# applied-ai-lab/genesis

Hardware: AMD Instinct MI355X
Metric: training images/sec (fwd+bwd+GECO step), GENESIS-V2 K=7 64x64 (higher is better)
Workload: dtype f32

## Files before the change

### genesis_amd/build.py

```python
import os
import os.path as osp
import subprocess
import sys

HERE = osp.dirname(osp.abspath(__file__))
CSRC = osp.join(HERE, 'csrc')
LIB = osp.join(HERE, 'libgenesis_hip.so')
SOURCES = ['gx_api.cpp', 'gx_comm.cpp', 'gx_conv.hip', 'gx_norm.hip', 'gx_attention.hip', 'gx_slots.hip', 'gx_optim.hip', 'gx_misc.hip', 'gx_gated.hip', 'gx_latent.hip', 'gx_dense.hip', 'gx_igemm.hip', 'gx_metrics.hip', 'gx_feed.hip', 'gx_wino.hip', 'gx_kq.hip', 'gx_bcast.hip', 'gx_sbp.hip', 'gx_wgq.hip', 'gx_wstrip.hip', 'gx_fid.hip', 'gx_tfrecord.cpp', 'gx_jpeg.cpp', 'gx_jpeg.hip', 'gx_png.cpp', 'gx_png.hip', 'gx_multid.hip']
HIPCC = os.environ.get('HIPCC', '/opt/rocm/bin/hipcc')
FLAGS = ['--offload-arch=gfx950', '-O3', '-std=c++17', '-fPIC', '-Wno-unused-value',
         '-Wno-pass-failed']


def _deps():
    d = [osp.join(CSRC, s) for s in SOURCES if osp.exists(osp.join(CSRC, s))]
    d += [osp.join(CSRC, 'gx_common.h'), osp.join(osp.dirname(HERE), 'include', 'genesis_hip.h'), osp.join(HERE, 'pk_peephole.py')]
    return d


def needs_build():
    if not osp.exists(LIB):
        return True
    t = osp.getmtime(LIB)
    return any(osp.getmtime(f) > t for f in _deps())


LLVM_BIN = os.environ.get('GENESIS_LLVM_BIN', '/opt/rocm/lib/llvm/bin')
TARGET = 'hipv4-amdgcn-amd-amdhsa--gfx950'


def _run(cmd, what):
    p = subprocess.run(cmd, stdout=subprocess.PIPE, stderr=subprocess.STDOUT)
    if p.returncode != 0:
        sys.stderr.write(' '.join(cmd) + '\n' + p.stdout.decode())
        raise RuntimeError('%s failed' % what)
    return p.stdout.decode()


def _compile_hip(src, obj):
    from genesis_amd import pk_peephole
    base = osp.splitext(obj)[0]
    asm, dev_o, hsaco, fatbin = base + '.dev.s', base + '.dev.o', base + '.hsaco', base + '.hipfb'
    _run([HIPCC] + FLAGS + ['--cuda-device-only', '-S', src, '-o', asm], 'device code generation of ' + src)
    with open(asm) as f:
        text, n = pk_peephole.rewrite(f.read())
    assert pk_peephole.count_bad(text) == 0
    with open(asm, 'w') as f:
        f.write(text)
    _run([osp.join(LLVM_BIN, 'clang'), '-x', 'assembler', '-target', 'amdgcn-amd-amdhsa', '-mcpu=gfx950', '-c', asm, '-o', dev_o],
         'assembling ' + asm)
    _run([osp.join(LLVM_BIN, 'lld'), '-flavor', 'gnu', '-m', 'elf64_amdgpu', '--no-undefined', '-shared', '-o', hsaco, dev_o],
         'linking ' + hsaco)
    _run([osp.join(LLVM_BIN, 'clang-offload-bundler'), '-type=o', '-bundle-align=4096',
          '-targets=host-x86_64-unknown-linux-gnu,' + TARGET, '-input=/dev/null', '-input=' + hsaco, '-output=' + fatbin],
         'bundling ' + fatbin)
    _run([HIPCC] + FLAGS + ['--cuda-host-only', '-Xclang', '-fcuda-include-gpubinary', '-Xclang', fatbin, '-c', src, '-o', obj],
         'host compilation of ' + src)
    for f in (asm, dev_o, hsaco, fatbin):
        os.remove(f)
    return n


def verify_objects(objs):
    from genesis_amd import pk_peephole
    import tempfile
    bad = {}
    with tempfile.TemporaryDirectory() as tmp:
        for obj in objs:
            import shutil
            shutil.copy(obj, osp.join(tmp, 'o.o'))
            subprocess.run([osp.join(LLVM_BIN, 'llvm-objdump'), '--offloading', 'o.o'], cwd=tmp, stdout=subprocess.PIPE,
                           stderr=subprocess.STDOUT)
            for f in os.listdir(tmp):
                if 'amdgcn' in f:
                    dis = subprocess.run([osp.join(LLVM_BIN, 'llvm-objdump'), '-d', osp.join(tmp, f)], stdout=subprocess.PIPE,
                                         stderr=subprocess.STDOUT)
                    n = pk_peephole.count_bad(dis.stdout.decode())
                    if n:
                        bad[osp.basename(obj)] = bad.get(osp.basename(obj), 0) + n
                os.remove(osp.join(tmp, f))
    return bad


def _jobs():
    n = os.environ.get('MAX_JOBS', '').strip()
    return max(1, int(n)) if n.isdigit() else min(16, len(SOURCES))


def build(force=False, verbose=True):
    if not force and not needs_build():
        return LIB
    from concurrent.futures import ThreadPoolExecutor
    objs, jobs = [], []
    with ThreadPoolExecutor(max_workers=_jobs()) as pool:
        for s in SOURCES:
            src = osp.join(CSRC, s)
            if not osp.exists(src):
                continue
            stem = osp.splitext(s)[0]
            obj = osp.join(CSRC, stem + ('_host.o' if s.endswith('.cpp') and stem + '.hip' in SOURCES else '.o'))
            objs.append(obj)
            if s.endswith('.hip'):
                if verbose:
                    print('%s %s -c %s -o %s   (device assembly through pk_peephole)' % (HIPCC, ' '.join(FLAGS), src, obj), flush=True)
                jobs.append((s, pool.submit(_compile_hip, src, obj)))
            else:
                cmd = [HIPCC] + FLAGS + ['-x', 'hip', '-c', src, '-o', obj]
                if verbose:
                    print(' '.join(cmd), flush=True)
                jobs.append((s, pool.submit(_run, cmd, 'hipcc on ' + s)))
        rewritten = {}
        for s, j in jobs:
            r = j.result()
            if isinstance(r, int) and r:
                rewritten[s] = r
    if verbose:
        print('pk_peephole: %d packed-fp32 instructions rewritten %s' % (sum(rewritten.values()), rewritten), flush=True)
    bad = verify_objects(objs)
    if bad:
        raise RuntimeError('affected packed-fp32 instruction forms left in the device code: %s' % bad)
    cmd = [HIPCC, '--offload-arch=gfx950', '-shared', '-fPIC', '-o', LIB] + objs + ['-ldl']
    if verbose:
        print(' '.join(cmd), flush=True)
    subprocess.check_call(cmd)
    return LIB


if __name__ == '__main__':
    print(build(force='--force' in sys.argv))
```

### genesis_amd/csrc/gx_dense.hip

```cpp
#include "gx_common.h"

namespace {

__device__ __forceinline__ float mask_factor(float m, bool elu) { return m > 0.f ? 1.f : (elu ? m + 1.f : 0.f); }

template <bool A_KC, bool B_KC, bool MASK, bool ROWSUM>
__device__ __forceinline__ void
dense_tile(float (*part)[256], float (*rpart)[16], int bx, int by, const float* __restrict__ a, int lda,
           const float* __restrict__ mask, const float* __restrict__ b, int ldb, const float* __restrict__ bias,
           int act, float* __restrict__ c, int ldc, int I, int J, int Kc, float* __restrict__ rs, int vec_a,
           int vec_b, float* __restrict__ rs2 = nullptr) {
    const int lane = threadIdx.x & 63, wave = threadIdx.x >> 6, nw = blockDim.x >> 6;
    const int idx = lane & 15, kq = lane >> 4;
    const int i0 = by * 16, j0 = bx * 16;
    const bool elu_mask = (act & 4) != 0;
    const bool acc_rs = (act & 8) != 0;
    act &= 3;
    const int ai = i0 + idx, bj = j0 + idx;
    const bool a_ok = ai < I, b_ok = bj < J;
    f32x4 acc = {0.f, 0.f, 0.f, 0.f};
    float rsum = 0.f;
#pragma unroll 2
    for (int k16 = wave * 16; k16 < Kc; k16 += nw * 16) {
        const int kb = k16 + 4 * kq;
        float av[4], bv[4];
        if (A_KC) {
            if (vec_a) {
                f32x4 t = {0.f, 0.f, 0.f, 0.f}, m = {1.f, 1.f, 1.f, 1.f};
                if (a_ok && kb < Kc) {
                    t = *reinterpret_cast<const f32x4*>(a + (size_t)ai * lda + kb);
                    if (MASK) m = *reinterpret_cast<const f32x4*>(mask + (size_t)ai * lda + kb);
                }
#pragma unroll
                for (int jj = 0; jj < 4; ++jj) av[jj] = MASK ? t[jj] * mask_factor(m[jj], elu_mask) : t[jj];
            } else {
#pragma unroll
                for (int jj = 0; jj < 4; ++jj) {
                    float t = 0.f;
                    if (a_ok && kb + jj < Kc) {
                        t = a[(size_t)ai * lda + kb + jj];
                        if (MASK) t *= mask_factor(mask[(size_t)ai * lda + kb + jj], elu_mask);
                    }
                    av[jj] = t;
                }
            }
        } else {
#pragma unroll
            for (int jj = 0; jj < 4; ++jj) {
                float t = 0.f;
                if (a_ok && kb + jj < Kc) {
                    t = a[(size_t)(kb + jj) * lda + ai];
                    if (MASK) t *= mask_factor(mask[(size_t)(kb + jj) * lda + ai], elu_mask);
                }
                av[jj] = t;
            }
        }
        if (B_KC) {
            if (vec_b) {
                f32x4 t = {0.f, 0.f, 0.f, 0.f};
                if (b_ok && kb < Kc) t = *reinterpret_cast<const f32x4*>(b + (size_t)bj * ldb + kb);
#pragma unroll
                for (int jj = 0; jj < 4; ++jj) bv[jj] = t[jj];
            } else {
#pragma unroll
                for (int jj = 0; jj < 4; ++jj)
                    bv[jj] = (b_ok && kb + jj < Kc) ? b[(size_t)bj * ldb + kb + jj] : 0.f;
            }
        } else {
#pragma unroll
            for (int jj = 0; jj < 4; ++jj)
                bv[jj] = (b_ok && kb + jj < Kc) ? b[(size_t)(kb + jj) * ldb + bj] : 0.f;
        }
#pragma unroll
        for (int jj = 0; jj < 4; ++jj) {
            acc = __builtin_amdgcn_mfma_f32_16x16x4f32(av[jj], bv[jj], acc, 0, 0, 0);
            if (ROWSUM) rsum += av[jj];
        }
    }
#pragma unroll
    for (int r = 0; r < 4; ++r) part[wave][(kq * 4 + r) * 16 + idx] = acc[r];
    if (ROWSUM) {
        rsum += __shfl_xor(rsum, 16, 64);
        rsum += __shfl_xor(rsum, 32, 64);
        if (kq == 0) rpart[wave][idx] = rsum;
    }
    __syncthreads();
    if (threadIdx.x < 256) {
        const int t = threadIdx.x;
        float s = part[0][t];
        for (int w = 1; w < nw; ++w) s += part[w][t];
        const int ci = i0 + (t >> 4), cj = j0 + (t & 15);
        if (ci < I && cj < J) {
            if (bias) s += bias[cj];
            if (act == 1) s = s > 0.f ? s : 0.f;
            if (act == 2) s += c[(size_t)ci * ldc + cj];
            if (act == 3) s = s > 0.f ? s : expm1f(s);
            c[(size_t)ci * ldc + cj] = s;
        }
    }
    if (ROWSUM && bx == 0 && threadIdx.x < 16 && i0 + (int)threadIdx.x < I) {
        float s = rpart[0][threadIdx.x];
        for (int w = 1; w < nw; ++w) s += rpart[w][threadIdx.x];
        if (acc_rs) { rs[i0 + threadIdx.x] += s; if (rs2) rs2[i0 + threadIdx.x] += s; }
        else { rs[i0 + threadIdx.x] = s; if (rs2) rs2[i0 + threadIdx.x] = s; }
    }
}

template <bool A_KC, bool B_KC, bool MASK, bool ROWSUM>
__global__ void __launch_bounds__(1024)
dense_kernel(const float* __restrict__ a, int lda, const float* __restrict__ mask, const float* __restrict__ b,
             int ldb, const float* __restrict__ bias, int act, float* __restrict__ c, int ldc, int I, int J, int Kc,
             float* __restrict__ rs, int vec_a, int vec_b, float* __restrict__ rs2) {
    __shared__ float part[16][256];
    __shared__ float rpart[16][16];
    dense_tile<A_KC, B_KC, MASK, ROWSUM>(part, rpart, blockIdx.x, blockIdx.y, a, lda, mask, b, ldb, bias, act, c, ldc,
                                         I, J, Kc, rs, vec_a, vec_b, rs2);
}

template <bool MASK, bool ROWSUM>
__global__ void __launch_bounds__(1024)
dense_bwd_pair_kernel(const float* __restrict__ g, int ldg, const float* __restrict__ y, const float* __restrict__ w,
                      const float* __restrict__ x, int ldx, float* __restrict__ dx, int lddx, int dx_act,
                      float* __restrict__ dw, float* __restrict__ db, float* __restrict__ db2, int M, int N, int K,
                      int gy_dx, int vec) {
    __shared__ float part[16][256];
    __shared__ float rpart[16][16];
    if ((int)blockIdx.y < gy_dx)
        dense_tile<true, false, MASK, false>(part, rpart, blockIdx.x, blockIdx.y, g, ldg, y, w, K, nullptr, dx_act & 7, dx,
                                             lddx, M, K, N, nullptr, vec, 0);
    else
        dense_tile<false, false, MASK, ROWSUM>(part, rpart, blockIdx.x, blockIdx.y - gy_dx, g, ldg, y, x, ldx, nullptr,
                                               (dx_act & 4) | ((dx_act & 16) ? 10 : 0), dw, K, N, K, M, db, 0, 0, db2);
}

__device__ __forceinline__ float sigmoid_f(float x) { return 1.f / (1.f + expf(-x)); }

__device__ __forceinline__ f32x4 lstm_load4(const float* p, bool coh) {
    if (!coh) return *reinterpret_cast<const f32x4*>(p);
    f32x4 v;
#pragma unroll
    for (int i = 0; i < 4; ++i) v[i] = __hip_atomic_load(p + i, __ATOMIC_RELAXED, __HIP_MEMORY_SCOPE_AGENT);
    return v;
}
__device__ __forceinline__ void lstm_store(float* p, float v, bool coh) {
    if (coh) __hip_atomic_store(p, v, __ATOMIC_RELAXED, __HIP_MEMORY_SCOPE_AGENT);
    else *p = v;
}

template <bool COH>
__device__ __forceinline__ void
lstm_fwd_body(float (&part)[4][4][256], const float* __restrict__ gx, const float* h_prev, const float* c_prev,
              const float* __restrict__ w_hh, const float* __restrict__ b_hh, int B, int H, float* act, float* c_out,
              float* h_out) {
    const int lane = threadIdx.x & 63, wave = threadIdx.x >> 6;
    const int idx = lane & 15, kq = lane >> 4;
    const int i0 = blockIdx.y * 16, j0 = blockIdx.x * 16;
    const bool a_ok = i0 + idx < B;
    f32x4 acc[4];
#pragma unroll
    for (int q = 0; q < 4; ++q) { acc[q][0] = 0.f; acc[q][1] = 0.f; acc[q][2] = 0.f; acc[q][3] = 0.f; }
    if (h_prev) {
        for (int k16 = wave * 16; k16 < H; k16 += 64) {
            const int kb = k16 + 4 * kq;
            f32x4 av = {0.f, 0.f, 0.f, 0.f};
            if (a_ok) av = lstm_load4(h_prev + (size_t)(i0 + idx) * H + kb, COH);
            f32x4 bv[4];
#pragma unroll
            for (int q = 0; q < 4; ++q)
                bv[q] = *reinterpret_cast<const f32x4*>(w_hh + (size_t)(q * H + j0 + idx) * H + kb);
#pragma unroll
            for (int jj = 0; jj < 4; ++jj)
#pragma unroll
                for (int q = 0; q < 4; ++q)
                    acc[q] = __builtin_amdgcn_mfma_f32_16x16x4f32(av[jj], bv[q][jj], acc[q], 0, 0, 0);
        }
    }
#pragma unroll
    for (int q = 0; q < 4; ++q)
#pragma unroll
        for (int r = 0; r < 4; ++r) part[wave][q][(kq * 4 + r) * 16 + idx] = acc[q][r];
    __syncthreads();
    const int t = threadIdx.x;
    const int b = i0 + (t >> 4), u = j0 + (t & 15);
    if (b < B) {
        float pre[4];
#pragma unroll
        for (int q = 0; q < 4; ++q) {
            float s = part[0][q][t];
#pragma unroll
            for (int w = 1; w < 4; ++w) s += part[w][q][t];
            pre[q] = s + gx[(size_t)b * 4 * H + q * H + u] + b_hh[q * H + u];
        }
        const float ig = sigmoid_f(pre[0]), fg = sigmoid_f(pre[1]), gg = tanhf(pre[2]), og = sigmoid_f(pre[3]);
        const float cp = c_prev ? c_prev[(size_t)b * H + u] : 0.f;
        const float cn = fg * cp + ig * gg;
        float* ar = act + (size_t)b * 4 * H + u;
        ar[0] = ig; ar[H] = fg; ar[2 * H] = gg; ar[3 * H] = og;
        c_out[(size_t)b * H + u] = cn;
        lstm_store(h_out + (size_t)b * H + u, og * tanhf(cn), COH);
    }
}

__global__ void __launch_bounds__(256)
lstm_step_fwd_kernel(const float* __restrict__ gx, const float* __restrict__ h_prev,
                     const float* __restrict__ c_prev, const float* __restrict__ w_hh,
                     const float* __restrict__ b_hh, int B, int H, float* __restrict__ act,
                     float* __restrict__ c_out, float* __restrict__ h_out) {
    __shared__ float part[4][4][256];
    lstm_fwd_body<false>(part, gx, h_prev, c_prev, w_hh, b_hh, B, H, act, c_out, h_out);
}

constexpr int kLstmSeqBar = 16;
constexpr int kLstmSeqMaxWg = 128;

__device__ __forceinline__ void lstm_grid_barrier(unsigned* bar, unsigned nwg) {
    asm volatile("s_waitcnt vmcnt(0)" ::: "memory");
    __syncthreads();
    if (threadIdx.x == 0) {
        __hip_atomic_fetch_add(bar, 1u, __ATOMIC_RELAXED, __HIP_MEMORY_SCOPE_AGENT);
        while (__hip_atomic_load(bar, __ATOMIC_RELAXED, __HIP_MEMORY_SCOPE_AGENT) < nwg) __builtin_amdgcn_s_sleep(1);
    }
    __syncthreads();
}

__device__ __forceinline__ void lstm_grid_finish(unsigned* bar, unsigned nwg) {
    if (threadIdx.x == 0) {
        const unsigned seen = __hip_atomic_fetch_add(bar + kLstmSeqBar - 1, 1u, __ATOMIC_RELAXED, __HIP_MEMORY_SCOPE_AGENT);
        if (seen == nwg - 1) {
            for (int i = 0; i < kLstmSeqBar; ++i) __hip_atomic_store(bar + i, 0u, __ATOMIC_RELAXED, __HIP_MEMORY_SCOPE_AGENT);
        }
    }
}

__global__ void __launch_bounds__(256)
lstm_seq_fwd_kernel(const float* __restrict__ gx, const float* __restrict__ w_hh, const float* __restrict__ b_hh, int T, int B,
                    int H, float* act, float* c, float* h, unsigned* bar) {
    __shared__ float part[4][4][256];
    const unsigned nwg = gridDim.x * gridDim.y;
    const size_t sh = (size_t)B * H;
    for (int t = 0; t < T; ++t) {
        if (t) lstm_grid_barrier(bar + (t - 1), nwg);
        lstm_fwd_body<true>(part, gx + (size_t)t * 4 * sh, t ? h + (size_t)(t - 1) * sh : nullptr, t ? c + (size_t)(t - 1) * sh : nullptr,
                            w_hh, b_hh, B, H, act + (size_t)t * 4 * sh, c + (size_t)t * sh, h + (size_t)t * sh);
    }
    lstm_grid_finish(bar, nwg);
}

template <bool COH>
__device__ __forceinline__ void
lstm_bwd_body(float (&part)[16][256], const float* __restrict__ g_h, const float* dgates_next, const float* __restrict__ w_hh,
              const float* __restrict__ act, const float* __restrict__ c, const float* __restrict__ c_prev, const float* dc_next,
              int B, int H, float* dgates, float* dc_prev) {
    const int lane = threadIdx.x & 63, wave = threadIdx.x >> 6, nw = blockDim.x >> 6;
    const int idx = lane & 15, kq = lane >> 4;
    const int i0 = blockIdx.y * 16, j0 = blockIdx.x * 16;
    const bool a_ok = i0 + idx < B;
    f32x4 acc = {0.f, 0.f, 0.f, 0.f};
    if (dgates_next) {
        const int Kc = 4 * H;
// ... 40 lines not shown
                     const float* __restrict__ c_prev, const float* __restrict__ dc_next, int B, int H,
                     float* __restrict__ dgates, float* __restrict__ dc_prev) {
    __shared__ float part[16][256];
    lstm_bwd_body<false>(part, g_h, dgates_next, w_hh, act, c, c_prev, dc_next, B, H, dgates, dc_prev);
}

__global__ void __launch_bounds__(1024)
lstm_seq_bwd_kernel(const float* __restrict__ g_h, const float* __restrict__ w_hh, const float* __restrict__ act,
                    const float* __restrict__ c, int T, int B, int H, float* dgates, float* dc2, unsigned* bar) {
    __shared__ float part[16][256];
    const unsigned nwg = gridDim.x * gridDim.y;
    const size_t sh = (size_t)B * H;
    for (int t = T - 1; t >= 0; --t) {
        if (t + 1 < T) lstm_grid_barrier(bar + t, nwg);
        lstm_bwd_body<true>(part, g_h + (size_t)t * sh, t + 1 < T ? dgates + (size_t)(t + 1) * 4 * sh : nullptr, w_hh,
                      act + (size_t)t * 4 * sh, c + (size_t)t * sh, t ? c + (size_t)(t - 1) * sh : nullptr,
                      t + 1 < T ? dc2 + (size_t)((t + 1) & 1) * sh : nullptr, B, H, dgates + (size_t)t * 4 * sh,
                      dc2 + (size_t)(t & 1) * sh);
    }
    lstm_grid_finish(bar, nwg);
}


constexpr int kNN_MR = 8;
__global__ void __launch_bounds__(256)
matmul_nn_fwd_kernel(const float* __restrict__ x, const float* __restrict__ w, float* __restrict__ y, int M, int N, int K) {
    const int n0 = (blockIdx.y * 256 + threadIdx.x) * 4;
    const int m0 = blockIdx.x * kNN_MR;
    if (n0 >= N) return;
    float4 acc[kNN_MR];
#pragma unroll
    for (int r = 0; r < kNN_MR; ++r) acc[r] = make_float4(0.f, 0.f, 0.f, 0.f);
    const float* xr[kNN_MR];
#pragma unroll
    for (int r = 0; r < kNN_MR; ++r) xr[r] = x + (size_t)(m0 + r < M ? m0 + r : M - 1) * K;
    for (int k = 0; k < K; ++k) {
        const float4 w4 = *reinterpret_cast<const float4*>(w + (size_t)k * N + n0);
#pragma unroll
        for (int r = 0; r < kNN_MR; ++r) {
            const float xv = xr[r][k];
            acc[r].x = fmaf(xv, w4.x, acc[r].x); acc[r].y = fmaf(xv, w4.y, acc[r].y);
            acc[r].z = fmaf(xv, w4.z, acc[r].z); acc[r].w = fmaf(xv, w4.w, acc[r].w);
        }
    }
#pragma unroll
    for (int r = 0; r < kNN_MR; ++r)
        if (m0 + r < M) *reinterpret_cast<float4*>(y + (size_t)(m0 + r) * N + n0) = acc[r];
}

constexpr int kNN_KC = 16;
__global__ void __launch_bounds__(256)
matmul_nn_dw_kernel(const float* __restrict__ x, const float* __restrict__ g, float* __restrict__ dw, int M, int N, int K) {
    __shared__ float4 red[3][kNN_KC][64];
    const int lane = threadIdx.x & 63, wave = threadIdx.x >> 6;
    const int n0 = (blockIdx.y * 64 + lane) * 4;
    const int k0 = blockIdx.x * kNN_KC;
    const bool n_ok = n0 < N;
    float4 acc[kNN_KC];
#pragma unroll
    for (int r = 0; r < kNN_KC; ++r) acc[r] = make_float4(0.f, 0.f, 0.f, 0.f);
    if (n_ok)
        for (int m = wave; m < M; m += 4) {
            const float4 g4 = *reinterpret_cast<const float4*>(g + (size_t)m * N + n0);
            const float* xm = x + (size_t)m * K;
#pragma unroll
            for (int r = 0; r < kNN_KC; ++r) {
                const float xv = xm[k0 + r < K ? k0 + r : K - 1];
                acc[r].x = fmaf(xv, g4.x, acc[r].x); acc[r].y = fmaf(xv, g4.y, acc[r].y);
                acc[r].z = fmaf(xv, g4.z, acc[r].z); acc[r].w = fmaf(xv, g4.w, acc[r].w);
            }
        }
    if (wave > 0) {
#pragma unroll
        for (int r = 0; r < kNN_KC; ++r) red[wave - 1][r][lane] = acc[r];
    }
    __syncthreads();
    if (wave == 0 && n_ok) {
#pragma unroll
        for (int r = 0; r < kNN_KC; ++r) {
            float4 v = acc[r];
#pragma unroll
            for (int w = 0; w < 3; ++w) {
                const float4 t = red[w][r][lane];
                v.x += t.x; v.y += t.y; v.z += t.z; v.w += t.w;
            }
            if (k0 + r < K) *reinterpret_cast<float4*>(dw + (size_t)(k0 + r) * N + n0) = v;
        }
    }
}

__global__ void __launch_bounds__(256)
matmul_nn_dx_kernel(const float* __restrict__ g, const float* __restrict__ w, float* __restrict__ part, int M, int N, int K,
                    int cols_per_chunk) {
    __shared__ float gs[32][68], ws[64][68];
    const int t = threadIdx.x;
    const int m0 = blockIdx.y * 32, k0 = blockIdx.z * 64;
    const int c_begin = blockIdx.x * cols_per_chunk;
    const int c_end = c_begin + cols_per_chunk < N ? c_begin + cols_per_chunk : N;
    const int mi = (t >> 4) * 2, ki = (t & 15) * 4;
    float acc[2][4] = {};
    for (int c0 = c_begin; c0 < c_end; c0 += 64) {
        for (int e = t; e < 32 * 16; e += 256) {
            const int r = e >> 4, q = (e & 15) * 4;
            float4 v = make_float4(0.f, 0.f, 0.f, 0.f);
            if (m0 + r < M && c0 + q < c_end) v = *reinterpret_cast<const float4*>(g + (size_t)(m0 + r) * N + c0 + q);
            *reinterpret_cast<float4*>(&gs[r][q]) = v;
        }
        for (int e = t; e < 64 * 16; e += 256) {
            const int r = e >> 4, q = (e & 15) * 4;
            float4 v = make_float4(0.f, 0.f, 0.f, 0.f);
            if (k0 + r < K && c0 + q < c_end) v = *reinterpret_cast<const float4*>(w + (size_t)(k0 + r) * N + c0 + q);
            *reinterpret_cast<float4*>(&ws[r][q]) = v;
        }
        __syncthreads();
#pragma unroll 4
        for (int c = 0; c < 64; c += 4) {
            float4 a[2], b[4];
#pragma unroll
            for (int i = 0; i < 2; ++i) a[i] = *reinterpret_cast<const float4*>(&gs[mi + i][c]);
#pragma unroll
            for (int j = 0; j < 4; ++j) b[j] = *reinterpret_cast<const float4*>(&ws[ki + j][c]);
#pragma unroll
            for (int i = 0; i < 2; ++i)
#pragma unroll
                for (int j = 0; j < 4; ++j)
                    acc[i][j] = fmaf(a[i].x, b[j].x, fmaf(a[i].y, b[j].y, fmaf(a[i].z, b[j].z, fmaf(a[i].w, b[j].w, acc[i][j]))));
        }
        __syncthreads();
    }
    float* o = part + (size_t)blockIdx.x * M * K;
#pragma unroll
    for (int i = 0; i < 2; ++i)
#pragma unroll
        for (int j = 0; j < 4; ++j)
            if (m0 + mi + i < M && k0 + ki + j < K) o[(size_t)(m0 + mi + i) * K + k0 + ki + j] = acc[i][j];
}

__global__ void __launch_bounds__(256)
matmul_nn_dx_reduce_kernel(const float* __restrict__ part, float* __restrict__ dx, int MK, int nchunk) {
    const int i = blockIdx.x * 256 + threadIdx.x;
    if (i >= MK) return;
    float s0 = 0.f, s1 = 0.f;
    int c = 0;
    for (; c + 1 < nchunk; c += 2) { s0 += part[(size_t)c * MK + i]; s1 += part[(size_t)(c + 1) * MK + i]; }
    if (c < nchunk) s0 += part[(size_t)c * MK + i];
    dx[i] = s0 + s1;
}

inline int matmul_nn_chunks(int N) {
    const int tiles = gx_ceil_div(N, 64);
    return tiles < 128 ? tiles : 128;
}

inline bool aligned16(const void* p) { return (reinterpret_cast<uintptr_t>(p) & 15) == 0; }
inline int dense_threads(int Kc) { return Kc >= 1024 ? 1024 : 256; }

}

extern "C" {

int gx_linear_fwd_ld(const float* x, int ldx, const float* w, const float* b, int act, float* y, int ldy, int M,
                     int N, int K, gx_stream_t stream) {
    GX_CHECK_ARG(x && w && y, "gx_linear_fwd: null pointer");
    GX_CHECK_ARG(M > 0 && N > 0 && K > 0, "gx_linear_fwd: bad M/N/K (%d,%d,%d)", M, N, K);
    GX_CHECK_ARG(ldx >= K && ldy >= N, "gx_linear_fwd: row strides (%d,%d) shorter than the rows (%d,%d)", ldx, ldy, K, N);
    GX_CHECK_ARG(act >= 0 && act <= 2, "gx_linear_fwd: act must be 0 (none), 1 (ReLU) or 2 (ELU)");
    if (act == 2) act = 3;
    hipStream_t s = (hipStream_t)stream;
    const int vec_w = (K % 4 == 0) && aligned16(w);
    const int vec_x = vec_w && (ldx % 4 == 0) && aligned16(x);
    {
        GxProf pf(KID_DENSE, s, 2.0 * M * N * K, 4.0 * ((double)M * K + (double)N * K + (double)M * N));
        hipLaunchKernelGGL((dense_kernel<true, true, false, false>), dim3(gx_ceil_div(N, 16), gx_ceil_div(M, 16)),
                           dim3(dense_threads(K)), 0, s, x, ldx, (const float*)nullptr, w, K, b, act, y, ldy, M, N, K,
                           (float*)nullptr, vec_x, vec_w, (float*)nullptr);
    }
    GX_CHECK_LAUNCH("gx_linear_fwd");
    return GX_OK;
}

int gx_linear_fwd(const float* x, const float* w, const float* b, int act, float* y, int M, int N, int K,
                  gx_stream_t stream) {
    return gx_linear_fwd_ld(x, K, w, b, act, y, N, M, N, K, stream);
}

int gx_linear_bwd_ex(const float* x, int ldx, const float* w, const float* y, const float* g, int ldg, int act,
                     float* dx, int lddx, int dx_accumulate, float* dw, float* db, float* db2, int M, int N, int K,
                     gx_stream_t stream) {
    GX_CHECK_ARG(x && w && g, "gx_linear_bwd: null pointer");
    GX_CHECK_ARG(M > 0 && N > 0 && K > 0, "gx_linear_bwd: bad M/N/K (%d,%d,%d)", M, N, K);
    GX_CHECK_ARG(ldx >= K && ldg >= N && (!dx || lddx >= K), "gx_linear_bwd: a row stride is shorter than its rows");
    GX_CHECK_ARG(act == 0 || ((act == 1 || act == 2) && y), "gx_linear_bwd: act 1 (ReLU) / 2 (ELU) needs the layer output y");
    GX_CHECK_ARG(dw || !db, "gx_linear_bwd: db is produced together with dw");
    GX_CHECK_ARG(db || !db2, "gx_linear_bwd: db2 is a second copy of db");
    hipStream_t s = (hipStream_t)stream;
    const int vec = (N % 4 == 0) && (ldg % 4 == 0) && aligned16(g) && (act == 0 || aligned16(y));
    GX_CHECK_ARG(dx_accumulate >= 0 && dx_accumulate <= 3, "gx_linear_bwd: dx_accumulate is a bit mask (1: dx, 2: dw / db)");
    const int elu = act == 2 ? 4 : 0;
    const int dwacc = (dx_accumulate & 2) ? 10 : 0;
    const int dx_act = ((dx_accumulate & 1) ? 2 : 0) | elu | ((dx_accumulate & 2) ? 16 : 0);
    if (act == 2) act = 1;
    if (dx && dw) {
        GxProf pf(KID_DENSE, s, 4.0 * M * N * K, 4.0 * (4.0 * M * N + 2.0 * N * K + 2.0 * M * K));
        const int gy_dx = gx_ceil_div(M, 16);
        const dim3 grid(gx_ceil_div(K, 16), gy_dx + gx_ceil_div(N, 16)), block(dense_threads(M > N ? M : N));
        const float* mask = act == 1 ? y : nullptr;
#define GX_PAIR(MASK, ROWSUM)                                                                                        \
        hipLaunchKernelGGL((dense_bwd_pair_kernel<MASK, ROWSUM>), grid, block, 0, s, g, ldg, mask, w, x, ldx, dx,    \
                           lddx, dx_act, dw, db, db2, M, N, K, gy_dx, vec)
        if (act == 1) { if (db) GX_PAIR(true, true); else GX_PAIR(true, false); }
        else          { if (db) GX_PAIR(false, true); else GX_PAIR(false, false); }
#undef GX_PAIR
        GX_CHECK_LAUNCH("gx_linear_bwd(dx+dw)");
        return GX_OK;
    }
    if (dx) {
        GxProf pf(KID_DENSE, s, 2.0 * M * N * K, 4.0 * (2.0 * M * N + (double)N * K + (double)M * K));
        const dim3 grid(gx_ceil_div(K, 16), gx_ceil_div(M, 16)), block(dense_threads(N));
        if (act == 1)
            hipLaunchKernelGGL((dense_kernel<true, false, true, false>), grid, block, 0, s, g, ldg, y, w, K,
                               (const float*)nullptr, dx_act & 7, dx, lddx, M, K, N, (float*)nullptr, vec, 0, (float*)nullptr);
        else
            hipLaunchKernelGGL((dense_kernel<true, false, false, false>), grid, block, 0, s, g, ldg,
                               (const float*)nullptr, w, K, (const float*)nullptr, dx_act & 7, dx, lddx, M, K, N,
                               (float*)nullptr, vec, 0, (float*)nullptr);
    }
    GX_CHECK_LAUNCH("gx_linear_bwd(dx)");
    if (dw) {
        GxProf pf(KID_DENSE, s, 2.0 * M * N * K, 4.0 * (2.0 * M * N + (double)M * K + (double)N * K));
        const dim3 grid(gx_ceil_div(K, 16), gx_ceil_div(N, 16)), block(dense_threads(M));
        if (act == 1) {
            if (db)
                hipLaunchKernelGGL((dense_kernel<false, false, true, true>), grid, block, 0, s, g, ldg, y, x, ldx,
                                   (const float*)nullptr, elu | dwacc, dw, K, N, K, M, db, 0, 0, db2);
            else
                hipLaunchKernelGGL((dense_kernel<false, false, true, false>), grid, block, 0, s, g, ldg, y, x, ldx,
                                   (const float*)nullptr, elu | dwacc, dw, K, N, K, M, (float*)nullptr, 0, 0, (float*)nullptr);
        } else {
            if (db)
                hipLaunchKernelGGL((dense_kernel<false, false, false, true>), grid, block, 0, s, g, ldg,
                                   (const float*)nullptr, x, ldx, (const float*)nullptr, dwacc, dw, K, N, K, M, db, 0, 0,
                                   db2);
            else
                hipLaunchKernelGGL((dense_kernel<false, false, false, false>), grid, block, 0, s, g, ldg,
                                   (const float*)nullptr, x, ldx, (const float*)nullptr, dwacc, dw, K, N, K, M,
                                   (float*)nullptr, 0, 0, (float*)nullptr);
        }
    }
    GX_CHECK_LAUNCH("gx_linear_bwd(dw)");
    return GX_OK;
}

int gx_linear_bwd(const float* x, const float* w, const float* y, const float* g, int act, float* dx, float* dw,
                  float* db, int M, int N, int K, gx_stream_t stream) {
    return gx_linear_bwd_ex(x, K, w, y, g, N, act, dx, K, 0, dw, db, nullptr, M, N, K, stream);
}

int gx_matmul_nn_fwd(const float* x, const float* w, float* y, int M, int N, int K, gx_stream_t stream) {
    GX_CHECK_ARG(x && w && y, "gx_matmul_nn_fwd: null pointer");
    GX_CHECK_ARG(M > 0 && N > 0 && K > 0 && (N % 4) == 0, "gx_matmul_nn_fwd: bad M/N/K (%d,%d,%d; N %% 4 == 0)", M, N, K);
    GX_CHECK_ARG(aligned16(w) && aligned16(y), "gx_matmul_nn_fwd: 16-byte alignment");
    hipStream_t s = (hipStream_t)stream;
    {
        GxProf pf(KID_DENSE, s, 2.0 * M * N * K, 4.0 * ((double)M * K + (double)N * K + (double)M * N));
        hipLaunchKernelGGL(matmul_nn_fwd_kernel, dim3(gx_ceil_div(M, kNN_MR), gx_ceil_div(N, 1024)), dim3(256), 0, s, x, w, y, M,
                           N, K);
    }
    GX_CHECK_LAUNCH("gx_matmul_nn_fwd");
    return GX_OK;
}

size_t gx_matmul_nn_bwd_ws_bytes(int M, int N, int K) {
    if (M <= 0 || N <= 0 || K <= 0) return 0;
    return (size_t)matmul_nn_chunks(N) * M * K * sizeof(float);
}

int gx_matmul_nn_bwd(const float* x, const float* w, const float* g, float* dx, float* dw, int M, int N, int K, void* ws,
                     size_t ws_bytes, gx_stream_t stream) {
    GX_CHECK_ARG(x && w && g, "gx_matmul_nn_bwd: null pointer");
    GX_CHECK_ARG(M > 0 && N > 0 && K > 0 && (N % 4) == 0, "gx_matmul_nn_bwd: bad M/N/K (%d,%d,%d; N %% 4 == 0)", M, N, K);
    GX_CHECK_ARG(aligned16(w) && aligned16(g) && (!dw || aligned16(dw)), "gx_matmul_nn_bwd: 16-byte alignment");
    hipStream_t s = (hipStream_t)stream;
    if (dw) {
        GxProf pf(KID_DENSE, s, 2.0 * M * N * K, 4.0 * ((double)M * K + (double)N * K + (double)M * N));
        hipLaunchKernelGGL(matmul_nn_dw_kernel, dim3(gx_ceil_div(K, kNN_KC), gx_ceil_div(N, 256)), dim3(256), 0, s, x, g, dw, M,
                           N, K);
        GX_CHECK_LAUNCH("gx_matmul_nn_bwd(dw)");
    }
    if (dx) {
        GX_CHECK_ARG(ws && ws_bytes >= gx_matmul_nn_bwd_ws_bytes(M, N, K), "gx_matmul_nn_bwd: workspace too small");
        const int nchunk = matmul_nn_chunks(N);
        const int cols = gx_round_up(gx_ceil_div(N, nchunk), 64);
        const int used = gx_ceil_div(N, cols);
        {
            GxProf pf(KID_DENSE, s, 2.0 * M * N * K, 4.0 * ((double)M * K + (double)N * K + (double)M * N));
            hipLaunchKernelGGL(matmul_nn_dx_kernel, dim3(used, gx_ceil_div(M, 32), gx_ceil_div(K, 64)), dim3(256), 0, s, g, w,
                               (float*)ws, M, N, K, cols);
        }
        GX_CHECK_LAUNCH("gx_matmul_nn_bwd(dx)");
        {
            GxProf pf(KID_SMALL_REDUCE, s, 0.0, 4.0 * (used + 1.0) * M * K);
            hipLaunchKernelGGL(matmul_nn_dx_reduce_kernel, dim3(gx_ceil_div(M * K, 256)), dim3(256), 0, s, (const float*)ws, dx,
                               M * K, used);
        }
        GX_CHECK_LAUNCH("gx_matmul_nn_bwd(dx reduce)");
    }
    return GX_OK;
}

// ... 76 lines not shown
```

### genesis_amd/csrc/gx_latent.hip

```cpp
#include "gx_common.h"

namespace {

constexpr float kHalfLog2Pi = 0.91893853320467274178f;

__device__ __forceinline__ float softplus_t(float x) {
    return x > 20.f ? x : log1pf(expf(x));
}
__device__ __forceinline__ float softplus_grad_t(float x) {
    if (x > 20.f) return 1.f;
    const float e = expf(x);
    return e / (e + 1.f);
}
__device__ __forceinline__ float sigmoid_t(float x) { return 1.f / (1.f + expf(-x)); }

__global__ void __launch_bounds__(256)
posterior_fwd_kernel(const float* __restrict__ zh, const float* __restrict__ eps, int B, int K, int D,
                     float* __restrict__ z, float* __restrict__ mu_o, float* __restrict__ sigma_o,
                     float* __restrict__ log_q, float* __restrict__ z2, int ldz2) {
    const int row = blockIdx.x * (blockDim.x >> 6) + (threadIdx.x >> 6);
    if (row >= K * B) return;
    const int lane = threadIdx.x & 63;
    const int k = row / B, b = row - k * B;
    const float* zr = zh + ((size_t)b * K + k) * 2 * D;
    double acc = 0.0;
    for (int d = lane; d < D; d += 64) {
        const float mu = zr[d];
        const float sg = softplus_t(zr[D + d] + 0.5f) + 1e-8f;
        const float zz = mu + sg * eps[(size_t)row * D + d];
        const float t = zz - mu;
        const float lp = -(t * t) / (2.f * (sg * sg)) - logf(sg) - kHalfLog2Pi;
        z[(size_t)row * D + d] = zz;
        if (z2) z2[(size_t)row * ldz2 + d] = zz;
        mu_o[(size_t)row * D + d] = mu;
        sigma_o[(size_t)row * D + d] = sg;
        acc += (double)lp;
    }
    acc = gx_wave_sum_d(acc);
    if (lane == 0) log_q[row] = (float)acc;
}

__global__ void __launch_bounds__(256)
posterior_bwd_kernel(const float* __restrict__ zh, const float* __restrict__ eps, const float* __restrict__ gz,
                     const float* __restrict__ gmu, const float* __restrict__ gsigma,
                     const float* __restrict__ glogq, int B, int K, int D, float* __restrict__ dzh,
                     const float* __restrict__ gz2, int ldgz2) {
    const int row = blockIdx.x * (blockDim.x >> 6) + (threadIdx.x >> 6);
    if (row >= K * B) return;
    const int lane = threadIdx.x & 63;
    const int k = row / B, b = row - k * B;
    const float* zr = zh + ((size_t)b * K + k) * 2 * D;
    float* dr = dzh + ((size_t)b * K + k) * 2 * D;
    const float gl = glogq ? glogq[row] : 0.f;
    for (int d = lane; d < D; d += 64) {
        const size_t i = (size_t)row * D + d;
        const float mu = zr[d];
        const float raw = zr[D + d] + 0.5f;
        const float sg = softplus_t(raw) + 1e-8f;
        const float e = eps[i];
        const float zz = mu + sg * e;
        const float t = zz - mu;
        const float var = sg * sg;
        const float dz = (gz ? gz[i] : 0.f) + (gz2 ? gz2[(size_t)row * ldgz2 + d] : 0.f) + gl * (-t / var);
        const float dmu = dz + gl * (t / var) + (gmu ? gmu[i] : 0.f);
        const float dsg = dz * e + gl * ((t * t) / (var * sg) - 1.f / sg) + (gsigma ? gsigma[i] : 0.f);
        dr[d] = dmu;
        dr[D + d] = dsg * softplus_grad_t(raw);
    }
}

__global__ void __launch_bounds__(256)
prior_logp_fwd_kernel(const float* __restrict__ z, const float* __restrict__ lin,
                      const float* __restrict__ log_q, int B, int K, int D, int first, float* __restrict__ log_p) {
    const int row = blockIdx.x * (blockDim.x >> 6) + (threadIdx.x >> 6);
    if (row >= K * B) return;
    const int lane = threadIdx.x & 63;
    const bool ar = lin != nullptr && row >= first;
    const float* lr = ar ? lin + (size_t)(row - first) * 2 * D : nullptr;
    double acc = 0.0;
    for (int d = lane; d < D; d += 64) {
        const float zz = z[(size_t)row * D + d];
        float lp;
        if (ar) {
            const float mu = tanhf(lr[d]);
            const float sg = sigmoid_t(lr[D + d] + 4.f) + 1e-4f;
            const float t = zz - mu;
            lp = -(t * t) / (2.f * (sg * sg)) - logf(sg) - kHalfLog2Pi;
        } else {
            lp = -(zz * zz) / 2.f - kHalfLog2Pi;
        }
        acc += (double)lp;
    }
    acc = gx_wave_sum_d(acc);
    if (lane == 0) log_p[row] = log_q ? log_q[row] - (float)acc : (float)acc;
}

__global__ void __launch_bounds__(256)
prior_sample_kernel(const float* __restrict__ lin, const float* __restrict__ eps, int B, int D, int tanh_mu,
                    float* __restrict__ z) {
    const int i = blockIdx.x * blockDim.x + threadIdx.x;
    if (i >= B * D) return;
    const int b = i / D, d = i - b * D;
    const float raw = lin[(size_t)b * 2 * D + d];
    const float mu = tanh_mu ? tanhf(raw) : raw;
    const float sg = sigmoid_t(lin[(size_t)b * 2 * D + D + d] + 4.f) + 1e-4f;
    z[i] = mu + sg * eps[i];
}

__global__ void __launch_bounds__(256)
prior_logp_bwd_kernel(const float* __restrict__ z, const float* __restrict__ lin, const float* __restrict__ glogp,
                      float sign, int B, int K, int D, int first, float* __restrict__ dz, float* __restrict__ dlin) {
    const int row = blockIdx.x * (blockDim.x >> 6) + (threadIdx.x >> 6);
    if (row >= K * B) return;
    const int lane = threadIdx.x & 63;
    const bool ar = lin != nullptr && row >= first;
    const float* lr = ar ? lin + (size_t)(row - first) * 2 * D : nullptr;
    float* dl = ar ? dlin + (size_t)(row - first) * 2 * D : nullptr;
    const float g = sign * glogp[row];
    for (int d = lane; d < D; d += 64) {
        const size_t i = (size_t)row * D + d;
        const float zz = z[i];
        if (ar) {
            const float mu = tanhf(lr[d]);
            const float s = sigmoid_t(lr[D + d] + 4.f);
            const float sg = s + 1e-4f;
            const float t = zz - mu;
            const float var = sg * sg;
            dz[i] = g * (-t / var);
            dl[d] = g * (t / var) * (1.f - mu * mu);
            dl[D + d] = g * ((t * t) / (var * sg) - 1.f / sg) * (s * (1.f - s));
        } else {
            dz[i] = g * (-zz);
        }
    }
}

__global__ void __launch_bounds__(256)
elbo_fwd_kernel(const float* __restrict__ err, const float* __restrict__ kl, const float* __restrict__ beta,
                int B, int R, float* __restrict__ out, float* __restrict__ tail, float* __restrict__ loss,
                float* __restrict__ d_err = nullptr, float* __restrict__ d_kl = nullptr) {
    __shared__ double red[2][4];
    if (d_err) {
        const float ge = 1.f / B, gk = *beta / B;
        for (int i = threadIdx.x; i < B; i += blockDim.x) d_err[i] = ge;
        if (d_kl) for (int i = threadIdx.x; i < R * B; i += blockDim.x) d_kl[i] = gk;
    }
    double se = 0.0, sk = 0.0;
    for (int i = threadIdx.x; i < B; i += blockDim.x) se += (double)err[i];
    for (int i = threadIdx.x; i < R * B; i += blockDim.x) sk += (double)kl[i];
    se = gx_wave_sum_d(se); sk = gx_wave_sum_d(sk);
    const int lane = threadIdx.x & 63, wave = threadIdx.x >> 6;
    if (lane == 0) { red[0][wave] = se; red[1][wave] = sk; }
    __syncthreads();
    if (threadIdx.x == 0) {
        const double e = ((red[0][0] + red[0][1]) + (red[0][2] + red[0][3])) / B;
        const double k = ((red[1][0] + red[1][1]) + (red[1][2] + red[1][3])) / B;
        const float ef = (float)e, kf = (float)k, bt = *beta;
        out[0] = ef + bt * kf; out[1] = ef + kf; out[2] = ef; out[3] = kf; out[4] = bt;
        if (tail) { tail[0] = ef; tail[1] = kf; }
        if (loss) loss[0] = out[0];
    }
}

__global__ void __launch_bounds__(256)
elbo_bwd_kernel(const float* __restrict__ g, const float* __restrict__ beta, int B, int R,
                float* __restrict__ d_err, float* __restrict__ d_kl) {
    const float ge = g[0] / B, gk = g[0] * (*beta) / B;
    const int i = blockIdx.x * blockDim.x + threadIdx.x;
    if (i < B) d_err[i] = ge;
    if (i < R * B) d_kl[i] = gk;
}

__global__ void __launch_bounds__(256)
pooled_head_fwd_kernel(const float* __restrict__ lin, const float* __restrict__ msum,
                       const float* __restrict__ fbias, const float* __restrict__ gamma,
                       const float* __restrict__ beta, float eps, int R, int C, float* __restrict__ y,
                       float* __restrict__ stats ) {
    const int row = blockIdx.x * (blockDim.x >> 6) + (threadIdx.x >> 6);
    if (row >= R) return;
    const int lane = threadIdx.x & 63;
    const float m = msum[row];
    const float den = m + 1e-5f;
    double s1 = 0.0, s2 = 0.0;
    for (int j = lane; j < C; j += 64) {
        const float o = (lin[(size_t)row * C + j] + m * fbias[j]) / den;
        s1 += (double)o; s2 += (double)o * o;
    }
    s1 = gx_wave_sum_d(s1); s2 = gx_wave_sum_d(s2);
    const double mean = s1 / C;
    double var = s2 / C - mean * mean;
    if (var < 0.0) var = 0.0;
    const float meanf = (float)mean, rstd = (float)(1.0 / sqrt(var + (double)eps));
    for (int j = lane; j < C; j += 64) {
        const float o = (lin[(size_t)row * C + j] + m * fbias[j]) / den;
        y[(size_t)row * C + j] = (o - meanf) * rstd * gamma[j] + beta[j];
    }
    if (lane == 0) { stats[2 * row] = meanf; stats[2 * row + 1] = rstd; }
}

__global__ void __launch_bounds__(256)
pooled_head_bwd_kernel(const float* __restrict__ lin, const float* __restrict__ msum,
                       const float* __restrict__ fbias, const float* __restrict__ gamma,
                       const float* __restrict__ stats, const float* __restrict__ g, int R, int C,
                       float* __restrict__ dlin, float* __restrict__ dmsum, float* __restrict__ cols) {
    const int row = blockIdx.x * (blockDim.x >> 6) + (threadIdx.x >> 6);
    if (row >= R) return;
    const int lane = threadIdx.x & 63;
    const float m = msum[row];
    const float den = m + 1e-5f;
    const float meanf = stats[2 * row], rstd = stats[2 * row + 1];
    double a = 0.0, b = 0.0;
    for (int j = lane; j < C; j += 64) {
        const float o = (lin[(size_t)row * C + j] + m * fbias[j]) / den;
        const float xh = (o - meanf) * rstd;
        const float dxh = g[(size_t)row * C + j] * gamma[j];
        a += (double)dxh; b += (double)dxh * xh;
    }
    a = gx_wave_sum_d(a); b = gx_wave_sum_d(b);
    const float k1 = (float)(a / C), k2 = (float)(b / C);
    double dm = 0.0;
    for (int j = lane; j < C; j += 64) {
        const float num = lin[(size_t)row * C + j] + m * fbias[j];
        const float o = num / den;
        const float xh = (o - meanf) * rstd;
        const float gv = g[(size_t)row * C + j];
        const float dobj = rstd * (gv * gamma[j] - k1 - xh * k2);
        dlin[(size_t)row * C + j] = dobj / den;
        dm += (double)dobj * ((double)fbias[j] / den - (double)num / ((double)den * den));
        float* cr = cols + (size_t)row * 3 * C;
        cr[j] = gv * xh; cr[C + j] = gv; cr[2 * C + j] = dobj * (m / den);
    }
    dm = gx_wave_sum_d(dm);
    if (lane == 0) dmsum[row] = (float)dm;
}

__global__ void __launch_bounds__(256)
pooled_head_cols_kernel(const float* __restrict__ cols, int R, int C, float* __restrict__ dgamma,
                        float* __restrict__ dbeta, float* __restrict__ dfbias) {
    __shared__ double red[8][32];
    const int cl = threadIdx.x & 31, rg = threadIdx.x >> 5;
    const int i = blockIdx.x * 32 + cl;
    double s = 0.0;
    if (i < 3 * C)
        for (int r = rg; r < R; r += 8) s += (double)cols[(size_t)r * 3 * C + i];
    red[rg][cl] = s;
    __syncthreads();
    if (rg == 0 && i < 3 * C) {
        double t = red[0][cl];
        for (int q = 1; q < 8; ++q) t += red[q][cl];
        const int which = i / C, j = i - which * C;
        (which == 0 ? dgamma : (which == 1 ? dbeta : dfbias))[j] = (float)t;
    }
}

int check_bkd(const char* name, int B, int K, int D) {
    GX_CHECK_ARG(B > 0 && K > 0 && D > 0, "%s: bad B/K/D (%d,%d,%d)", name, B, K, D);
    return GX_OK;
}

}

extern "C" {

int gx_latent_posterior_fwd(const float* zh, const float* eps, int B, int K, int D, float* z, float* mu,
                            float* sigma, float* log_q, gx_stream_t stream) {
    return gx_latent_posterior_fwd_ex(zh, eps, B, K, D, z, mu, sigma, log_q, nullptr, 0, stream);
}

int gx_latent_posterior_fwd_ex(const float* zh, const float* eps, int B, int K, int D, float* z, float* mu,
                               float* sigma, float* log_q, float* z2, int ldz2, gx_stream_t stream) {
    int rc = check_bkd("gx_latent_posterior_fwd", B, K, D);
    if (rc) return rc;
    GX_CHECK_ARG(zh && eps && z && mu && sigma && log_q, "gx_latent_posterior_fwd: null pointer");
    GX_CHECK_ARG(!z2 || ldz2 >= D, "gx_latent_posterior_fwd_ex: ldz2 (%d) < D (%d)", ldz2, D);
    hipStream_t s = (hipStream_t)stream;
    {
        GxProf pf(KID_LATENT, s, 0.0, 4.0 * (6.0 * K * B * D + K * B));
        hipLaunchKernelGGL(posterior_fwd_kernel, dim3(gx_ceil_div(K * B, 4)), dim3(256), 0, s, zh, eps, B, K, D, z,
                           mu, sigma, log_q, z2, ldz2);
    }
    GX_CHECK_LAUNCH("gx_latent_posterior_fwd");
    return GX_OK;
}

int gx_latent_posterior_bwd(const float* zh, const float* eps, const float* gz, const float* gmu,
                            const float* gsigma, const float* glogq, int B, int K, int D, float* dzh,
                            gx_stream_t stream) {
    return gx_latent_posterior_bwd_ex(zh, eps, gz, gmu, gsigma, glogq, nullptr, 0, B, K, D, dzh, stream);
}

int gx_latent_posterior_bwd_ex(const float* zh, const float* eps, const float* gz, const float* gmu,
                               const float* gsigma, const float* glogq, const float* gz2, int ldgz2, int B, int K,
                               int D, float* dzh, gx_stream_t stream) {
    int rc = check_bkd("gx_latent_posterior_bwd", B, K, D);
    if (rc) return rc;
    GX_CHECK_ARG(zh && eps && dzh, "gx_latent_posterior_bwd: null pointer");
    GX_CHECK_ARG(!gz2 || ldgz2 >= D, "gx_latent_posterior_bwd_ex: ldgz2 (%d) < D (%d)", ldgz2, D);
    hipStream_t s = (hipStream_t)stream;
    {
        GxProf pf(KID_LATENT, s, 0.0, 4.0 * (8.0 * K * B * D + K * B));
        hipLaunchKernelGGL(posterior_bwd_kernel, dim3(gx_ceil_div(K * B, 4)), dim3(256), 0, s, zh, eps, gz, gmu,
                           gsigma, glogq, B, K, D, dzh, gz2, ldgz2);
    }
    GX_CHECK_LAUNCH("gx_latent_posterior_bwd");
    return GX_OK;
}

int gx_latent_prior_logp_fwd(const float* z, const float* lin, const float* log_q, int B, int K, int D,
                             float* out, gx_stream_t stream) {
    return gx_latent_prior_logp_fwd_ex(z, lin, log_q, B, K, D, 0, out, stream);
}

int gx_latent_prior_logp_fwd_ex(const float* z, const float* lin, const float* log_q, int B, int K, int D, int all_slots,
                                float* out, gx_stream_t stream) {
    float* log_p = out;
    int rc = check_bkd("gx_latent_prior_logp_fwd", B, K, D);
    if (rc) return rc;
    GX_CHECK_ARG(z && log_p, "gx_latent_prior_logp_fwd: null pointer");
    hipStream_t s = (hipStream_t)stream;
    {
        GxProf pf(KID_LATENT, s, 0.0, 4.0 * (3.0 * K * B * D + K * B));
        hipLaunchKernelGGL(prior_logp_fwd_kernel, dim3(gx_ceil_div(K * B, 4)), dim3(256), 0, s, z, lin, log_q, B, K,
                           D, all_slots ? 0 : B, log_p);
    }
    GX_CHECK_LAUNCH("gx_latent_prior_logp_fwd");
    return GX_OK;
}

int gx_latent_prior_sample(const float* lin, const float* eps, int B, int D, float* z, gx_stream_t stream) {
    return gx_latent_prior_sample_ex(lin, eps, B, D, 1, z, stream);
}

int gx_latent_prior_sample_ex(const float* lin, const float* eps, int B, int D, int tanh_mu, float* z,
                              gx_stream_t stream) {
    GX_CHECK_ARG(lin && eps && z && B > 0 && D > 0, "gx_latent_prior_sample: bad arguments");
    hipStream_t s = (hipStream_t)stream;
    {
        GxProf pf(KID_LATENT, s, 0.0, 16.0 * B * D);
        hipLaunchKernelGGL(prior_sample_kernel, dim3(gx_ceil_div(B * D, 256)), dim3(256), 0, s, lin, eps, B, D, tanh_mu,
                           z);
    }
    GX_CHECK_LAUNCH("gx_latent_prior_sample");
    return GX_OK;
}

int gx_latent_prior_logp_bwd(const float* z, const float* lin, const float* g_out, int kl_mode, int B, int K,
                             int D, float* dz, float* dlin, gx_stream_t stream) {
    return gx_latent_prior_logp_bwd_ex(z, lin, g_out, kl_mode, B, K, D, 0, dz, dlin, stream);
}

int gx_latent_prior_logp_bwd_ex(const float* z, const float* lin, const float* g_out, int kl_mode, int B, int K,
                                int D, int all_slots, float* dz, float* dlin, gx_stream_t stream) {
    const float* glogp = g_out;
    int rc = check_bkd("gx_latent_prior_logp_bwd", B, K, D);
    if (rc) return rc;
    GX_CHECK_ARG(z && glogp && dz, "gx_latent_prior_logp_bwd: null pointer");
    GX_CHECK_ARG((lin == nullptr) == (dlin == nullptr), "gx_latent_prior_logp_bwd: lin and dlin go together");
    hipStream_t s = (hipStream_t)stream;
    {
        GxProf pf(KID_LATENT, s, 0.0, 4.0 * (6.0 * K * B * D + K * B));
        hipLaunchKernelGGL(prior_logp_bwd_kernel, dim3(gx_ceil_div(K * B, 4)), dim3(256), 0, s, z, lin, glogp,
                           kl_mode ? -1.f : 1.f, B, K, D, all_slots ? 0 : B, dz, dlin);
    }
    GX_CHECK_LAUNCH("gx_latent_prior_logp_bwd");
    return GX_OK;
}

int gx_elbo_fwd(const float* err, const float* kl, const float* beta, int B, int R, float* out, float* tail,
                float* loss, gx_stream_t stream) {
    GX_CHECK_ARG(err && beta && out, "gx_elbo_fwd: null pointer");
    GX_CHECK_ARG(B > 0 && R >= 0 && (R == 0 || kl), "gx_elbo_fwd: bad B/R (%d,%d) or missing kl", B, R);
    hipStream_t s = (hipStream_t)stream;
    {
        GxProf pf(KID_LATENT, s, 0.0, 4.0 * (B + (double)R * B));
        hipLaunchKernelGGL(elbo_fwd_kernel, dim3(1), dim3(256), 0, s, err, kl, beta, B, R, out, tail, loss);
    }
    GX_CHECK_LAUNCH("gx_elbo_fwd");
    return GX_OK;
}

int gx_elbo_fwd_grads(const float* err, const float* kl, const float* beta, int B, int R, float* out, float* tail,
                      float* loss, float* d_err, float* d_kl, gx_stream_t stream) {
    GX_CHECK_ARG(err && beta && out && d_err, "gx_elbo_fwd_grads: null pointer");
    GX_CHECK_ARG(B > 0 && R >= 0 && (R == 0 || (kl && d_kl)), "gx_elbo_fwd_grads: bad B/R (%d,%d) or missing kl / d_kl", B, R);
    hipStream_t s = (hipStream_t)stream;
    {
        GxProf pf(KID_LATENT, s, 0.0, 8.0 * (B + (double)R * B));
        hipLaunchKernelGGL(elbo_fwd_kernel, dim3(1), dim3(256), 0, s, err, kl, beta, B, R, out, tail, loss, d_err, d_kl);
    }
    GX_CHECK_LAUNCH("gx_elbo_fwd_grads");
    return GX_OK;
}

int gx_elbo_bwd(const float* g_loss, const float* beta, int B, int R, float* d_err, float* d_kl,
                gx_stream_t stream) {
    GX_CHECK_ARG(g_loss && beta && d_err, "gx_elbo_bwd: null pointer");
    GX_CHECK_ARG(B > 0 && R >= 0 && (R == 0 || d_kl), "gx_elbo_bwd: bad B/R (%d,%d) or missing d_kl", B, R);
    hipStream_t s = (hipStream_t)stream;
    const int n = R > 0 ? R * B : B;
    {
        GxProf pf(KID_LATENT, s, 0.0, 4.0 * (B + (double)R * B));
        hipLaunchKernelGGL(elbo_bwd_kernel, dim3(gx_ceil_div(n, 256)), dim3(256), 0, s, g_loss, beta, B, R, d_err,
                           d_kl);
    }
    GX_CHECK_LAUNCH("gx_elbo_bwd");
// ... 44 lines not shown
```

### genesis_amd/functions.py

```python
import os

import torch
import torch.nn.functional as F

from . import _lib
from . import autostep as _auto
from . import hip_ops as hip
from . import precision as _precision

GROUPS = 8
EPS = 1e-5

class _StepState(object):
    __slots__ = ('direct_param_grads', 'direct_written', 'async_wgrad', 'side_stream', 'keep_alive', 'early_flush')

    def __init__(self):
        self.direct_param_grads = False
        self.direct_written = set()
        self.async_wgrad = False
        self.side_stream = None
        self.keep_alive = []
        self.early_flush = None


# ... 823 lines not shown
                else:
                    dw = _wgrad_paired(h, dy, gw)
                pre = None
                if l >= 2 and hip.conv3x3_dgrad_act_supported(dy.shape[0], w.shape[1], w.shape[0], dy.shape[2], dy.shape[3]):
                    gbp = _gout(params[2 * l - 1])
                    wp = params[2 * l - 2]
                    lazy = wp.shape[0] == wp.shape[1] and _quad_ok(h.shape[0], wp.shape[1], h.shape[2], h.shape[3])
                    pre = hip.conv3x3_dgrad_act(dy, w, h, act, gbp, want_dbias=not lazy, amax_in=am, tap=True) + (gbp,)
                    am = hip.take_amax()
                else:
                    da = hip.conv3x3_dgrad(dy, w, amax_in=am)
                    am = None
            grads[2 * l], grads[2 * l + 1] = _ret(gw, dw), _ret(gb, db)
        return (dz, None, None, None) + tuple(grads)


def _quad_ok(N, C, H, W):
    return hip.conv3x3_wgrad_quad_supported(N, C, H, W)


def _wgrad_paired(h, dy, gw, gb=None):
    N, Ci, Co = h.shape[0], h.shape[1], dy.shape[1]
    if Ci == Co and hip.conv3x3_wgrad_quad_supported(N, Ci, h.shape[2], h.shape[3]):
        dw = hip.conv3x3_wgrad_quad(h, dy, out=gw, dbias_out=gb)
        return None if gw is not None else dw
    assert gb is None, 'the bias gradient rides on the four-image weight gradient only'
    if N % 2 or Ci > 32 or Co > 32 or Ci != Co or Ci % 8:
        return hip.conv3x3_wgrad(h, dy, out=gw)
    d64 = hip.conv3x3_wgrad(h.view(N // 2, 2 * Ci, *h.shape[2:]), dy.view(N // 2, 2 * Co, *dy.shape[2:]))
    dw = d64[:Co, :Ci] + d64[Co:, Ci:]
    if gw is not None:
        gw.copy_(dw)
        return None
    return dw


@ctx_bound
class MixtureWFn(torch.autograd.Function):

    @staticmethod
    def forward(ctx, x, dec, log_w, K, std1, std2, pixel_bound):
        x, dec, log_w = x.contiguous(), dec.contiguous(), log_w.contiguous()
        err, recon, x_r = hip.mixture_w_fwd(x, dec, log_w, K, std1, std2, pixel_bound)
        ctx.save_for_backward(x, dec, log_w)
        ctx.cfg = (K, std1, std2, pixel_bound)
        ctx.set_materialize_grads(False)
        return err, recon, x_r

    @staticmethod
    def backward(ctx, g_err, g_recon, g_x_r):
        x, dec, log_w = ctx.saved_tensors
        K, std1, std2, pixel_bound = ctx.cfg
        extra, extra_w = _fold_output_grads(dec, K, pixel_bound, g_recon, g_x_r, None, log_w)
        if g_err is None:
            if extra is not None:
                return None, extra, extra_w, None, None, None, None
            g_err = x.new_zeros(x.shape[0])
        ddec, dlog_w = hip.mixture_w_bwd(x, dec, log_w, g_err.contiguous(), K, std1, std2, pixel_bound)
        if extra is not None:
            ddec += extra
            if extra_w is not None:
                dlog_w += extra_w
        return None, ddec, dlog_w, None, None, None, None


def _c(t):
    return None if t is None else t.contiguous()


@ctx_bound
class PosteriorFn(torch.autograd.Function):

    @staticmethod
    def forward(ctx, zh, eps):
        zh, eps = zh.contiguous(), eps.contiguous()
        ctx.set_materialize_grads(False)
        ctx.save_for_backward(zh, eps)
        return hip.latent_posterior_fwd(zh, eps)

    @staticmethod
    def backward(ctx, gz, gmu, gsigma, glogq):
        zh, eps = ctx.saved_tensors
        return hip.latent_posterior_bwd(zh, eps, _c(gz), _c(gmu), _c(gsigma), _c(glogq)), None


@ctx_bound
class PriorLogPFn(torch.autograd.Function):

    @staticmethod
    def forward(ctx, z, lin, log_q=None, all_slots=False):
        z = z.contiguous()
        lin = None if lin is None else lin.contiguous()
        log_q = None if log_q is None else log_q.contiguous()
        ctx.save_for_backward(z, lin)
        ctx.kl_mode = log_q is not None
        ctx.all_slots = bool(all_slots)
        return hip.latent_prior_logp_fwd(z, lin, log_q, all_slots)

    @staticmethod
    def backward(ctx, g):
        z, lin = ctx.saved_tensors
        g = g.contiguous()
        dz, dlin = hip.latent_prior_logp_bwd(z, lin, g, ctx.kl_mode, ctx.all_slots)
        return dz, dlin, (g if ctx.kl_mode else None), None


@ctx_bound
class ElboFn(torch.autograd.Function):

    @staticmethod
    def forward(ctx, err, kl, beta, tail):
        err = err.contiguous()
        kl = None if kl is None else kl.contiguous()
        ctx.beta = beta
        ctx.dims = (err.numel(), 0 if kl is None else kl.numel() // err.numel())
        ctx.kl_shape = None if kl is None else kl.shape
        loss, out5 = hip.elbo_fwd(err, kl, beta, tail)
        ctx.mark_non_differentiable(out5)
        ctx.set_materialize_grads(False)
        return loss, out5

    @staticmethod
    def backward(ctx, g, _unused):
        B, R = ctx.dims
        d_err, d_kl = hip.elbo_bwd(g.contiguous(), ctx.beta, B, R)
        return d_err, (d_kl.view(ctx.kl_shape) if d_kl is not None else None), None, None


@ctx_bound
class PooledHeadFn(torch.autograd.Function):

    @staticmethod
    def forward(ctx, lin, msum, fbias, gamma, beta, eps):
        shape = lin.shape
        lin2 = lin.contiguous().view(-1, shape[-1])
        msum1 = msum.contiguous().view(-1)
        y, stats = hip.pooled_head_fwd(lin2, msum1, fbias, gamma, beta, eps)
        ctx.save_for_backward(lin2, msum1, stats)
        ctx.params = (fbias, gamma, beta)
        ctx.shapes = (shape, msum.shape)
        return y.view(shape)

    @staticmethod
    def backward(ctx, g):
        lin2, msum1, stats = ctx.saved_tensors
        fbias, gamma, beta = ctx.params
        outs = (_gout(fbias), _gout(gamma), _gout(beta))
        dlin, dmsum, dfb, dga, dbe = hip.pooled_head_bwd(lin2, msum1, fbias, gamma, stats,
                                                         g.contiguous().view(lin2.shape), out=outs)
        return (dlin.view(ctx.shapes[0]), dmsum.view(ctx.shapes[1]), _ret(outs[0], dfb), _ret(outs[1], dga),
                _ret(outs[2], dbe), None)


@ctx_bound
class SBPScanFn(torch.autograd.Function):

    @staticmethod
    def forward(ctx, logits, log_s0, last_scope):
        logits = logits.contiguous()
        log_s0 = None if log_s0 is None else log_s0.contiguous()
        ctx.save_for_backward(logits)
        ctx.last_scope = bool(last_scope)
        ctx.has_s0 = log_s0 is not None
        ctx.set_materialize_grads(False)
        return hip.sbp_scan_fwd(logits, log_s0, last_scope)

    @staticmethod
    def backward(ctx, g_m, g_s):
        logits, = ctx.saved_tensors
        want_s0 = ctx.has_s0 and ctx.needs_input_grad[1]
        g_logits, g_s0 = hip.sbp_scan_bwd(logits, _c(g_m), _c(g_s), ctx.last_scope, want_s0)
        return g_logits, g_s0, None


@ctx_bound
class CategoricalKLFn(torch.autograd.Function):

    @staticmethod
    def forward(ctx, log_m, log_m_r):
        log_m, log_m_r = log_m.contiguous(), log_m_r.contiguous()
        ctx.save_for_backward(log_m, log_m_r)
        return hip.categorical_kl_fwd(log_m, log_m_r)

    @staticmethod
    def backward(ctx, g):
        log_m, log_m_r = ctx.saved_tensors
        g_m, g_r = hip.categorical_kl_bwd(log_m, log_m_r, g.contiguous(), ctx.needs_input_grad[1])
        return g_m, g_r


@ctx_bound
class MaskReconFn(torch.autograd.Function):

    @staticmethod
    def forward(ctx, dec, log_m_r):
        ctx.save_for_backward(log_m_r)
        ctx.C = dec.shape[1]
        return log_m_r.view_as(log_m_r)

    @staticmethod
    def backward(ctx, g):
        log_m_r, = ctx.saved_tensors
        return hip.logsoftmax_k_bwd(log_m_r, g.contiguous(), ctx.C), None


@ctx_bound
class LSTMCellFn(torch.autograd.Function):

    @staticmethod
    def forward(ctx, inp, h_prev, c_prev, w_ih, w_hh, b_ih, b_hh):
        inp = inp.contiguous()
        B = inp.shape[0]
        H = w_hh.shape[1]
        gx = hip.linear_fwd(inp, w_ih, b_ih)
        act = torch.empty(B, 4 * H, device=inp.device)
        c = torch.empty(B, H, device=inp.device)
        h = torch.empty(B, H, device=inp.device)
        hp = None if h_prev is None else h_prev.contiguous()
        cp = None if c_prev is None else c_prev.contiguous()
        hip.lstm_step_fwd(gx, hp, cp, w_hh, b_hh, act, c, h)
        ctx.save_for_backward(inp, hp, cp, act, c)
        ctx.params = (w_ih, w_hh, b_ih, b_hh)
        ctx.set_materialize_grads(False)
        return h, c

    @staticmethod
    def backward(ctx, g_h, g_c):
        inp, hp, cp, act, c = ctx.saved_tensors
        w_ih, w_hh, b_ih, b_hh = ctx.params
        B, H = c.shape
        dev = inp.device
        if g_h is None:
            g_h = torch.zeros(B, H, device=dev)
        dgates = torch.empty(B, 4 * H, device=dev)
        dc_prev = torch.empty(B, H, device=dev)
        hip.lstm_step_bwd(g_h.contiguous(), None, w_hh, act, c, cp, _c(g_c), dgates, dc_prev)
        outs = [_gout_acc(p) for p in (w_ih, w_hh, b_ih, b_hh)]
        acc = outs[0][1]
        if any(o is None for o, _ in outs) or any(a != acc for _, a in outs):
            outs, acc = [(None, False)] * 4, False
        o_wih, o_whh, o_bih, o_bhh = (o for o, _ in outs)
        dinp, dw_ih, db = hip.linear_bwd(inp, w_ih, None, dgates, None, need_dx=ctx.needs_input_grad[0],
                                         out_dw=o_wih, out_db=o_bih, out_db2=o_bhh, accumulate_dw=acc)
        if hp is not None:
            dh_prev, dw_hh, _ = hip.linear_bwd(hp, w_hh, None, dgates, None, need_dx=True, need_db=False, out_dw=o_whh,
                                               accumulate_dw=acc)
        else:
            dh_prev = None
            dw_hh = torch.zeros_like(w_hh) if o_whh is None else (o_whh if acc else o_whh.zero_())
        return (dinp, dh_prev, dc_prev if cp is not None else None, _ret(o_wih, dw_ih), _ret(o_whh, dw_hh),
                _ret(o_bih, db), _ret(o_bhh, db))


@ctx_bound
class LatentSBPPosteriorFn(torch.autograd.Function):

    @staticmethod
    def forward(ctx, h, eps, w_m, b_m, w_v, b_v, w_ih, w_hh, b_ih, b_hh, w_lin, b_lin):
        h, eps = h.contiguous(), eps.contiguous()
        K, B, D = eps.shape
        F_, T, H = h.shape[1], K - 1, w_hh.shape[1]
        dev = h.device
        lin = torch.empty(K, B, 2 * D, device=dev)
        z, mu, sigma = (torch.empty(K, B, D, device=dev) for _ in range(3))
        log_q = torch.empty(K, B, device=dev)
        inp = torch.empty(max(T, 1), B, F_ + D, device=dev)
        if T:
            inp[:, :, :F_] = h
        act = torch.empty(max(T, 1), B, 4 * H, device=dev)
        c = torch.empty(max(T, 1), B, H, device=dev)
        hs = torch.empty(max(T, 1), B, H, device=dev)
        hip.linear_fwd(h, w_m, b_m, None, out=lin[0][:, :D])
        hip.linear_fwd(h, w_v, b_v, None, out=lin[0][:, D:])
        for k in range(K):
            if k:
                t = k - 1
                gx = hip.linear_fwd(inp[t], w_ih, b_ih)
                hip.lstm_step_fwd(gx, hs[t - 1] if t else None, c[t - 1] if t else None, w_hh, b_hh, act[t], c[t], hs[t])
                hip.linear_fwd(hs[t], w_lin, b_lin, None, out=lin[k])
            hip.latent_posterior_step_fwd(lin[k], eps[k], z[k], mu[k], sigma[k], log_q[k],
                                          inp[k][:, F_:] if k < T else None)
        ctx.save_for_backward(h, eps, lin, inp, act, c, hs)
        ctx.params = (w_m, b_m, w_v, b_v, w_ih, w_hh, b_ih, b_hh, w_lin, b_lin)
        ctx.set_materialize_grads(False)
        return z, mu, sigma, log_q

    @staticmethod
    def backward(ctx, gz, gmu, gsigma, glogq):
        h, eps, lin, inp, act, c, hs = ctx.saved_tensors
        w_m, b_m, w_v, b_v, w_ih, w_hh, b_ih, b_hh, w_lin, b_lin = ctx.params
        K, B, D = eps.shape
        F_, T, H = h.shape[1], K - 1, w_hh.shape[1]
        dev = h.device
        gz, gmu, gsigma, glogq = _c(gz), _c(gmu), _c(gsigma), _c(glogq)
        dlin = torch.empty(K, B, 2 * D, device=dev)
        dinp = torch.empty(max(T, 1), B, F_ + D, device=dev)
        dgates = torch.empty(max(T, 1), B, 4 * H, device=dev)
        dhs = torch.empty(B, H, device=dev)
        dc = [torch.empty(B, H, device=dev), torch.empty(B, H, device=dev)]

        def sl(g, k):
            return None if g is None else g[k]
        for k in reversed(range(K)):
            hip.latent_posterior_step_bwd(lin[k], eps[k], sl(gz, k), sl(gmu, k), sl(gsigma, k), sl(glogq, k),
                                          dinp[k][:, F_:] if k < T else None, dlin[k])
            if k:
# ... 266 lines not shown
```

### genesis_amd/genesisv2_config.py

```python
import math

import numpy as np
import torch
import torch.nn as nn
import torch.nn.functional as F
from torch.distributions.normal import Normal

from genesis_amd import autostep
from genesis_amd import compat as _compat

_compat.install()

from attrdict import AttrDict
from forge import flags

from genesis_amd import functions as fn
from genesis_amd.lazy import Lazy, LazyAttrDict, SlotList
from genesis_amd import hip_ops as hip

flags.DEFINE_integer('feat_dim', 64, 'Number of features and latents.')
flags.DEFINE_string('kernel', 'gaussian', '{laplacian, gaussian, epanechnikov')
flags.DEFINE_boolean('semiconv', True, 'Use semi-convolutional embeddings.')
flags.DEFINE_boolean('dynamic_K', False, 'Dynamic K.')
flags.DEFINE_boolean('klm_loss', False, 'KL mask regulariser.')
# ... 97 lines not shown
            sigma_init = 1.0 / (np.sqrt(K_steps) * np.log(2))
        elif kernel == 'gaussian':
            sigma_init = 1.0 / (K_steps * np.log(2))
        elif kernel == 'epanechnikov':
            sigma_init = 2.0 / K_steps
        else:
            raise ValueError('No valid kernel.')
        self.kernel = kernel
        self.colour_dim = colour_dim
        self.log_sigma = nn.Parameter(torch.tensor(sigma_init).log())
        self.semiconv = semiconv
        if semiconv:
            self.colour_head = _SemiConvParams(feat_dim, colour_dim)
        else:
            self.colour_head = nn.Conv2d(feat_dim, colour_dim, 1)


class GenesisV2(nn.Module):

    def __init__(self, cfg):
        super().__init__()
        self.K_steps = cfg.K_steps
        self.img_size = cfg.img_size
        self.pixel_bound = _cfg_get(cfg, 'pixel_bound', True)
        self.feat_dim = cfg.feat_dim
        self.klm_loss = _cfg_get(cfg, 'klm_loss', False)
        self.detach_mr_in_klm = _cfg_get(cfg, 'detach_mr_in_klm', True)
        self.dynamic_K = _cfg_get(cfg, 'dynamic_K', False)
        self.debug = _cfg_get(cfg, 'debug', False)
        self.multi_gpu = _cfg_get(cfg, 'multi_gpu', False)
        D = cfg.feat_dim
        self.encoder = _UNetParams(int(np.log2(cfg.img_size) - 1), cfg.img_size, min(D, 64), 3, D)
        self.att_process = _ICSBPParams(_cfg_get(cfg, 'kernel', 'gaussian'), self.K_steps, D,
                                        _cfg_get(cfg, 'semiconv', True))
        self.seg_head = _ConvGNReLU(D, D)
        self.feat_head = nn.Sequential(_ConvGNReLU(D, D), nn.Conv2d(D, 2 * D, 1))
        self.z_head = nn.Sequential(nn.LayerNorm(2 * D), nn.Linear(2 * D, 2 * D), nn.ReLU(inplace=True),
                                    nn.Linear(2 * D, 2 * D))
        c = D
        cm = min(c, 64)
        self.decoder_module = nn.Sequential(
            nn.Identity(),
            nn.ConvTranspose2d(D + 2, c, 5, 2, 2, 1), nn.GroupNorm(8, c), nn.ReLU(inplace=True),
            nn.ConvTranspose2d(c, c, 5, 2, 2, 1), nn.GroupNorm(8, c), nn.ReLU(inplace=True),
            nn.ConvTranspose2d(c, cm, 5, 2, 2, 1), nn.GroupNorm(8, cm), nn.ReLU(inplace=True),
            nn.ConvTranspose2d(cm, cm, 5, 2, 2, 1), nn.GroupNorm(8, cm), nn.ReLU(inplace=True),
            nn.Conv2d(cm, 4, 1))
        self.autoreg_prior = _cfg_get(cfg, 'autoreg_prior', True)
        self.prior_lstm, self.prior_linear = None, None
        if self.autoreg_prior and self.K_steps > 1:
            self.prior_lstm = nn.LSTM(D, 4 * D)
            self.prior_linear = nn.Linear(4 * D, 2 * D)
        assert _cfg_get(cfg, 'pixel_std1', 0.7) == _cfg_get(cfg, 'pixel_std2', 0.7)
        self.std = _cfg_get(cfg, 'pixel_std1', 0.7)
        self._grids = {}

    def _grid(self, device):
        key = str(device)
        if key not in self._grids:
            S, cd = self.img_size, self.att_process.colour_dim
            uv = torch.cat((torch.zeros(1, cd - 2, S, S), pixel_coords(S)), 1)[0].contiguous()
            dec_coords = pixel_coords(self.img_size // 16).contiguous()
            self._grids[key] = (uv.to(device), dec_coords.to(device))
        return self._grids[key]

    def _decoder_params(self):
        p = []
        for ci, gi in ((1, 2), (4, 5), (7, 8), (10, 11)):
            p.extend((self.decoder_module[ci].weight, self.decoder_module[ci].bias,
                      self.decoder_module[gi].weight, self.decoder_module[gi].bias))
        p.extend((self.decoder_module[13].weight, self.decoder_module[13].bias))
        return p

    def _decode(self, z_kbd, x=None, grad_through_masks=False):
        K, B, D = z_kbd.shape
        _, dec_coords = self._grid(z_kbd.device)
        dec = fn.DecoderFn.apply(z_kbd.reshape(K * B, D), dec_coords, *self._decoder_params())
        if x is None:
            x = torch.zeros(B, 3, self.img_size, self.img_size, device=z_kbd.device)
        err, recon, x_r, log_m_r = fn.MixtureFn.apply(x, dec, K, float(self.std), bool(self.pixel_bound))
        if grad_through_masks:
            log_m_r = fn.MaskReconFn.apply(dec, log_m_r)
        return err, recon, x_r, log_m_r

    def _prior_hidden(self, z_kbd):
        K, B, D = z_kbd.shape
        L = self.prior_lstm
        return fn.LSTMFn.apply(z_kbd[:-1], L.weight_ih_l0, L.weight_hh_l0, L.bias_ih_l0, L.bias_hh_l0)

    def _component_kl(self, z, log_q):
        lin = None
        if self.prior_lstm is not None:
            if z.shape[0] > 1:
                L, P = self.prior_lstm, self.prior_linear
                return fn.ARPriorKLFn.apply(z, log_q, L.weight_ih_l0, L.weight_hh_l0, L.bias_ih_l0, L.bias_hh_l0,
                                            P.weight, P.bias)
            lin = fn.linear(self._prior_hidden(z), self.prior_linear.weight, self.prior_linear.bias)
        return fn.PriorLogPFn.apply(z, lin, log_q)

    noise = None

    def forward(self, x, rand_pixel=None, eps=None, seed_idx=None):
        if x.is_cuda:
            if rand_pixel is None and eps is None and seed_idx is None:
                t = autostep.graph_forward(self, x)
                if t is not None:
                    return self._assemble(t)
            autostep.arm(self, x if (rand_pixel is None and eps is None and seed_idx is None) else None)
        return self._assemble(self._compute(x, rand_pixel, eps, seed_idx))

    def _compute(self, x, rand_pixel=None, eps=None, seed_idx=None):
        B, _, H, W = x.shape
        K, D = self.K_steps, self.feat_dim
        dev = x.device
        uv, _ = self._grid(dev)
        enc_feat = fn.UNetEncoderFn.apply(x, self.encoder.num_blocks, 8, *self.encoder.flat_params())
        if rand_pixel is None and eps is None and getattr(self, 'noise', None) is not None:
            rand_pixel, eps = self.noise((B, 1, H, W), (K, B, D), dev)
        if rand_pixel is None:
            rand_pixel = torch.rand(B, 1, H, W, device=dev)
        ap = self.att_process
        if ap.semiconv:
            cw, cb, gate, addend = ap.colour_head.conv.weight, ap.colour_head.conv.bias, ap.colour_head.gate.gate, uv
        else:
            cw, cb, gate, addend = ap.colour_head.weight, ap.colour_head.bias, None, None
        seg_params = self.seg_head.params()
        min_mass = 20.0 if self.dynamic_K else 0.0
        f = None
        if fn.heads_pairable(enc_feat, seg_params[0], cw, self.feat_head[0].params()[0]):
            res = fn.SegFeatHeadsFn.apply(enc_feat, *seg_params, cw, cb, gate, addend, ap.log_sigma, rand_pixel, K,
                                          ap.kernel, seed_idx, min_mass, *self.feat_head[0].params())
            res, f = res[:-1], res[-1]
        elif fn.seg_head_fusable(enc_feat, seg_params[0], cw):
            res = fn.SegICSBPFn.apply(enc_feat, *seg_params, cw, cb, gate, addend, ap.log_sigma, rand_pixel, K, ap.kernel,
                                      seed_idx, min_mass)
        else:
            seg = fn.ConvGNReLUFn.apply(enc_feat, *seg_params)
            res = fn.ICSBPFn.apply(seg, cw, cb, gate, addend, ap.log_sigma, rand_pixel, K, ap.kernel, seed_idx, min_mass)
        log_m, log_s, colour, seeds, idx = res[:5]
        dyn_batched = False
        if self.dynamic_K:
            if B == 1:
                n = int(res[5][0])
                K = n + 1
                log_m, log_s = log_m[:K], log_s[:K]
                seeds, idx = seeds[:min(n + 1, self.K_steps - 1)], idx[:min(n + 1, self.K_steps - 1)]
                if eps is not None:
                    eps = eps[:K]
            else:
                dyn_batched = True
        if f is None:
            f = fn.ConvGNReLUFn.apply(enc_feat, *self.feat_head[0].params())
        S, msum = fn.MaskPoolFn.apply(f, log_m)
        ln = self.z_head[0]
        zh = fn.PooledHeadFn.apply(fn.linear(S, self.feat_head[1].weight), msum, self.feat_head[1].bias,
                                   ln.weight, ln.bias, ln.eps)
        if eps is None:
            eps = torch.randn(K, B, D, device=dev)
        zh = fn.linear(zh, self.z_head[1].weight, self.z_head[1].bias, 'relu')
        zh = fn.linear(zh, self.z_head[3].weight, self.z_head[3].bias)
        z, mu, sigma, log_q = fn.PosteriorFn.apply(zh, eps)
        err, recon, x_r, log_m_r = self._decode(z, x, self.klm_loss and not self.detach_mr_in_klm)
        kl = self._component_kl(z, log_q)
        t = dict(err=err, kl=kl, recon=recon, log_m=log_m, log_s=log_s, x_r=x_r, log_m_r=log_m_r, colour=colour, seeds=seeds,
                 idx=idx, mu=mu, sigma=sigma, z=z)
        if self.klm_loss:
            t['kl_m'] = fn.CategoricalKLFn.apply(log_m, log_m_r.detach() if self.detach_mr_in_klm else log_m_r)
        t['dyn_batched'] = dyn_batched
        return t

    def _assemble(self, t):
        err, kl, recon, log_m, log_s, x_r, log_m_r = t['err'], t['kl'], t['recon'], t['log_m'], t['log_s'], t['x_r'], t['log_m_r']
        colour, seeds, idx, mu, sigma, z, dyn_batched = t['colour'], t['seeds'], t['idx'], t['mu'], t['sigma'], t['z'], t['dyn_batched']
        ap = self.att_process
        uv, _ = self._grid(recon.device)
        losses = AttrDict()
        losses['err'] = err
        log_m_k = list(log_m.unbind(0))
        log_s_k = None if dyn_batched else list(log_s.unbind(0))
        x_r_k = list(x_r.unbind(0))
        log_m_r_k = list(log_m_r.unbind(0))
        if 'kl_m' in t:
            losses['kl_m'] = t['kl_m']
        losses['kl_l_k'] = SlotList(kl.unbind(0), stacked=kl)

        stats = LazyAttrDict(
            recon=recon, log_m_k=log_m_k, log_s_k=log_s_k, x_r_k=x_r_k, log_m_r_k=log_m_r_k,
            mx_r_k=Lazy(lambda: list((x_r * log_m_r.exp()).unbind(0))),
            instance_seg=Lazy(lambda: torch.argmax(log_m.squeeze(2), dim=0)),
            instance_seg_r=Lazy(lambda: torch.argmax(log_m_r.squeeze(2), dim=0)))
        att_stats = LazyAttrDict()
        att_stats.update({'colour': colour,
                          'delta': Lazy(lambda: colour[:, -2:] - uv[-2:]) if ap.semiconv else None,
                          'seeds': list(seeds.unbind(0)), 'seed_idx': list(idx.unbind(0))})
        comp_stats = AttrDict(mu_k=list(mu.unbind(0)), sigma_k=list(sigma.unbind(0)), z_k=list(z.unbind(0)),
                              kl_l_k=[], q_z_k=[Normal(m, s, validate_args=False)
                                                for m, s in zip(mu.unbind(0), sigma.unbind(0))])
        if self.multi_gpu:
            del comp_stats['q_z_k']
        if dyn_batched:
            att_stats = None
        return recon, losses, stats, att_stats, comp_stats

    def decode_latents(self, z_k):
        _, recon, x_r, log_m_r = self._decode(torch.stack(list(z_k), 0))
        return recon, list(x_r.unbind(0)), list(log_m_r.unbind(0))

    @torch.no_grad()
    def sample(self, batch_size, K_steps=None, eps=None):
        K_steps = self.K_steps if K_steps is None else K_steps
        dev = self.decoder_module[13].weight.device
        D = self.feat_dim
        if eps is None:
            eps = torch.randn(K_steps, batch_size, D, device=dev)
        eps = eps.to(dev).contiguous()
        assert eps.shape == (K_steps, batch_size, D)
        if self.autoreg_prior and self.prior_lstm is not None:
            z_k = [eps[0]]
            w_ih, w_hh = self.prior_lstm.weight_ih_l0, self.prior_lstm.weight_hh_l0
            b_ih, b_hh = self.prior_lstm.bias_ih_l0, self.prior_lstm.bias_hh_l0
            H = w_hh.shape[1]
            h_prev = c_prev = None
            for k in range(1, K_steps):
                gx = hip.linear_fwd(z_k[-1].contiguous(), w_ih, b_ih)
                act = torch.empty(batch_size, 4 * H, device=dev)
                c = torch.empty(batch_size, H, device=dev)
                h = torch.empty(batch_size, H, device=dev)
                hip.lstm_step_fwd(gx, h_prev, c_prev, w_hh, b_hh, act, c, h)
                lin = hip.linear_fwd(h, self.prior_linear.weight, self.prior_linear.bias)
                z_k.append(hip.latent_prior_sample(lin, eps[k]))
                h_prev, c_prev = h, c
        else:
            z_k = list(eps.unbind(0))
        recon, x_r_k, log_m_r_k = self.decode_latents(z_k)
        stats = AttrDict(x_k=x_r_k, log_m_k=log_m_r_k, mx_k=[x * m.exp() for x, m in zip(x_r_k, log_m_r_k)],
                         z_k=z_k)
        return recon, stats

    def get_features(self, image_batch):
        with torch.no_grad():
            _, _, _, _, comp_stats = self.forward(image_batch)
            return torch.cat(comp_stats.z_k, dim=1)
```

### genesis_amd/hip_ops.py

```python
import ctypes
import os

import torch

from . import _lib
from ._lib import GenesisHipError

F32 = torch.float32
KERNELS = {'gaussian': 0, 'laplacian': 1, 'epanechnikov': 2}


def _chk(t, name, dtype=F32):
    if t is None:
        return
    if not t.is_cuda:
        raise GenesisHipError('%s: the HIP hot path needs device tensors (got %s); there is no CPU fallback'
                              % (name, t.device))
    if t.dtype != dtype:
        raise GenesisHipError('%s: expected %s, got %s' % (name, dtype, t.dtype))
    if not t.is_contiguous():
        raise GenesisHipError('%s: tensor must be contiguous' % name)


def _p(t):
# ... 1072 lines not shown
    _chk(z, 'prior.z'); _chk(lin, 'prior.lin'); _chk(log_q, 'prior.log_q')
    K, B, D = z.shape
    if lin is not None and tuple(lin.shape) != (K if all_slots else K - 1, B, 2 * D):
        raise GenesisHipError('latent_prior_logp_fwd: lin must be [%s,B,2D]' % ('K' if all_slots else 'K-1'))
    out = torch.empty(K, B, dtype=F32, device=z.device)
    _lib.call('gx_latent_prior_logp_fwd_ex', _p(z), _p(lin), _p(log_q), B, K, D, int(bool(all_slots)), _p(out), _stream())
    return out


def latent_prior_sample(lin, eps, tanh_mu=True):
    _chk(lin, 'prior_sample.lin'); _chk(eps, 'prior_sample.eps')
    B, D = eps.shape
    assert lin.shape == (B, 2 * D)
    z = torch.empty(B, D, dtype=F32, device=eps.device)
    _lib.call('gx_latent_prior_sample_ex', _p(lin), _p(eps), B, D, int(bool(tanh_mu)), _p(z), _stream())
    return z


def latent_prior_logp_bwd(z, lin, g_out, kl_mode=False, all_slots=False):
    _chk(g_out, 'prior_bwd.g_out')
    K, B, D = z.shape
    dz = torch.empty_like(z)
    dlin = torch.empty_like(lin) if lin is not None else None
    _lib.call('gx_latent_prior_logp_bwd_ex', _p(z), _p(lin), _p(g_out), int(kl_mode), B, K, D, int(bool(all_slots)), _p(dz),
              _p(dlin), _stream())
    return dz, dlin


def elbo_fwd(err, kl, beta, tail=None):
    _chk(err, 'elbo.err'); _chk(kl, 'elbo.kl'); _chk(beta, 'elbo.beta'); _chk(tail, 'elbo.tail')
    B = err.numel()
    R = 0 if kl is None else kl.numel() // B
    out = torch.empty(5, dtype=F32, device=err.device)
    loss = torch.empty(1, dtype=F32, device=err.device)
    _lib.call('gx_elbo_fwd', _p(err), _p(kl), _p(beta), B, R, _p(out), _p(tail), _p(loss), _stream())
    return loss, out


def elbo_fwd_grads(err, kl, beta, tail=None):
    _chk(err, 'elbo.err'); _chk(kl, 'elbo.kl'); _chk(beta, 'elbo.beta'); _chk(tail, 'elbo.tail')
    B = err.numel()
    R = 0 if kl is None else kl.numel() // B
    out = torch.empty(5, dtype=F32, device=err.device)
    d_err = torch.empty_like(err)
    d_kl = torch.empty_like(kl) if kl is not None else None
    _lib.call('gx_elbo_fwd_grads', _p(err), _p(kl), _p(beta), B, R, _p(out), _p(tail), None, _p(d_err), _p(d_kl), _stream())
    return out, d_err, d_kl


def elbo_bwd(g_loss, beta, B, R):
    _chk(g_loss, 'elbo_bwd.g')
    d_err = torch.empty(B, dtype=F32, device=g_loss.device)
    d_kl = torch.empty(R, B, dtype=F32, device=g_loss.device) if R else None
    _lib.call('gx_elbo_bwd', _p(g_loss), _p(beta), B, R, _p(d_err), _p(d_kl), _stream())
    return d_err, d_kl


def pooled_head_fwd(lin, msum, fbias, gamma, beta, eps):
    for t, n in ((lin, 'lin'), (msum, 'msum'), (fbias, 'fbias'), (gamma, 'gamma'), (beta, 'beta')):
        _chk(t, 'pooled_head.' + n)
    R, C = lin.shape
    y = torch.empty_like(lin)
    stats = torch.empty(R, 2, dtype=F32, device=lin.device)
    _lib.call('gx_pooled_head_fwd', _p(lin), _p(msum), _p(fbias), _p(gamma), _p(beta), float(eps), R, C, _p(y),
              _p(stats), _stream())
    return y, stats


def pooled_head_bwd(lin, msum, fbias, gamma, stats, g, out=(None, None, None)):
    _chk(g, 'pooled_head_bwd.g')
    R, C = lin.shape
    dev = lin.device
    dlin = torch.empty_like(lin)
    dmsum = torch.empty(R, dtype=F32, device=dev)
    dfb, dga, dbe = [o if o is not None else torch.empty(C, dtype=F32, device=dev) for o in out]
    nb = _lib.query('gx_pooled_head_bwd_ws_bytes', R, C)
    ws = _ws(nb, dev)
    _lib.call('gx_pooled_head_bwd', _p(lin), _p(msum), _p(fbias), _p(gamma), _p(stats), _p(g), R, C, _p(dlin),
              _p(dmsum), _p(dfb), _p(dga), _p(dbe), _p(ws), ws.numel(), _stream())
    return dlin, dmsum, dfb, dga, dbe


def _rows(t, name):
    if t.dim() != 2 or t.stride(1) != 1 or t.stride(0) < t.shape[1] or t.dtype != F32 or not t.is_cuda:
        raise GenesisHipError('%s: needs a float32 device matrix with contiguous rows, got %s strides %s'
                              % (name, tuple(t.shape), tuple(t.stride())))
    return t.stride(0)


def bcast_deconv_pack(w, b, coords):
    _chk(w, 'bcast_deconv.w'); _chk(b, 'bcast_deconv.b'); _chk(coords, 'bcast_deconv.coords')
    D, Cout, d = w.shape[0] - 2, w.shape[1], coords.shape[-1]
    if tuple(w.shape[2:]) != (5, 5) or coords.numel() != 2 * d * d or D <= 0:
        raise GenesisHipError('bcast_deconv_pack: w %s / coords %s' % (tuple(w.shape), tuple(coords.shape)))
    rows = Cout * 4 * d * d
    wz = torch.empty(rows, D, dtype=F32, device=w.device)
    bias = torch.empty(rows, dtype=F32, device=w.device)
    _lib.call('gx_bcast_deconv5x5s2_pack', _p(w), _p(b), _p(coords), D, Cout, d, _p(wz), _p(bias), _stream())
    return wz, bias


def bcast_deconv_unpack(dwz, dbias, coords, Cout, out_dw=None, out_db=None, want_db=False):
    _chk(dwz, 'bcast_deconv.dwz'); _chk(dbias, 'bcast_deconv.dbias'); _chk(coords, 'bcast_deconv.coords')
    _chk(out_dw, 'bcast_deconv.out_dw'); _chk(out_db, 'bcast_deconv.out_db')
    D, d = dwz.shape[1], coords.shape[-1]
    dw = out_dw if out_dw is not None else torch.empty(D + 2, Cout, 5, 5, dtype=F32, device=dwz.device)
    db = out_db if out_db is not None else (torch.empty(Cout, dtype=F32, device=dwz.device) if want_db else None)
    _lib.call('gx_bcast_deconv5x5s2_unpack', _p(dwz), _p(dbias), _p(coords), D, Cout, d, _p(dw), _p(db), _stream())
    return dw, db


def linear_fwd(x, w, b=None, act=None, out=None):
    _chk(w, 'linear.w'); _chk(b, 'linear.b')
    ldx = _rows(x, 'linear.x')
    M, K = x.shape
    N = w.shape[0]
    if w.shape[1] != K:
        raise GenesisHipError('linear_fwd: x is [%d,%d] but w is %s' % (M, K, tuple(w.shape)))
    y = torch.empty(M, N, dtype=F32, device=x.device) if out is None else out
    ldy = _rows(y, 'linear.out')
    if tuple(y.shape) != (M, N):
        raise GenesisHipError('linear_fwd: out is %s, expected (%d, %d)' % (tuple(y.shape), M, N))
    _lib.call('gx_linear_fwd_ld', _p(x), ldx, _p(w), _p(b), ACTS[act], _p(y), ldy, M, N, K, _stream())
    _probe_act(y, b, act)
    return y


def linear_bwd(x, w, y, g, act=None, need_dx=True, need_dw=True, need_db=True, out_dw=None, out_db=None,
               out_db2=None, accumulate_dx=None, accumulate_dw=False, out_dx=None):
    assert not accumulate_dw or out_dw is not None
    M, K = x.shape
    N = w.shape[0]
    dev = x.device
    ldx, ldg = _rows(x, 'linear_bwd.x'), _rows(g, 'linear_bwd.g')
    if y is not None and _rows(y, 'linear_bwd.y') != ldg:
        raise GenesisHipError('linear_bwd: y and g must share a row stride')
    if accumulate_dx is not None:
        dx = accumulate_dx
    elif out_dx is not None:
        dx = out_dx
    else:
        dx = torch.empty(M, K, dtype=F32, device=dev) if need_dx else None
    if dx is not None and tuple(dx.shape) != (M, K):
        raise GenesisHipError('linear_bwd: dx is %s, expected (%d, %d)' % (tuple(dx.shape), M, K))
    lddx = _rows(dx, 'linear_bwd.dx') if dx is not None else K
    dw = (out_dw if out_dw is not None else torch.empty(N, K, dtype=F32, device=dev)) if need_dw else None
    db = (out_db if out_db is not None else torch.empty(N, dtype=F32, device=dev)) if (need_db and need_dw) else None
    _lib.call('gx_linear_bwd_ex', _p(x), ldx, _p(w), _p(y), _p(g), ldg, ACTS[act], _p(dx), lddx,
              int(accumulate_dx is not None) | (2 if accumulate_dw else 0), _p(dw), _p(db),
              _p(out_db2 if db is not None else None), M, N, K, _stream())
    return dx, dw, db


def matmul_nn_fwd(x, w):
    _chk(x, 'matmul_nn.x'); _chk(w, 'matmul_nn.w')
    M, K = x.shape
    if w.shape[0] != K:
        raise GenesisHipError('matmul_nn_fwd: x is [%d,%d] but w is %s' % (M, K, tuple(w.shape)))
    y = torch.empty(M, w.shape[1], dtype=F32, device=x.device)
    _lib.call('gx_matmul_nn_fwd', _p(x), _p(w), _p(y), M, w.shape[1], K, _stream())
    return y


def matmul_nn_bwd(x, w, g, need_dx=True, out_dw=None, need_dw=True):
    _chk(x, 'matmul_nn_bwd.x'); _chk(w, 'matmul_nn_bwd.w'); _chk(g, 'matmul_nn_bwd.g')
    M, K = x.shape
    N = w.shape[1]
    dx = torch.empty(M, K, dtype=F32, device=x.device) if need_dx else None
    dw = (out_dw if out_dw is not None else torch.empty(K, N, dtype=F32, device=x.device)) if need_dw else None
    nb = _lib.query('gx_matmul_nn_bwd_ws_bytes', M, N, K) if need_dx else 0
    ws = _ws(nb, x.device) if need_dx else None
    _lib.call('gx_matmul_nn_bwd', _p(x), _p(w), _p(g), _p(dx), _p(dw), M, N, K, _p(ws), nb, _stream())
    return dx, dw


def logsoftmax_k_fwd(dec, K):
    _chk(dec, 'logsoftmax_k_fwd.dec')
    KB, C, H, W = dec.shape
    B = KB // K
    out = torch.empty(K, B, 1, H, W, dtype=F32, device=dec.device)
    _lib.call('gx_logsoftmax_k_fwd', _p(dec), K, B, H * W, C, _p(out), _stream())
    return out


def lstm_step_fwd(gx, h_prev, c_prev, w_hh, b_hh, act, c, h):
    B, H4 = gx.shape
    for t, n in ((gx, 'gx'), (h_prev, 'h_prev'), (c_prev, 'c_prev'), (w_hh, 'w_hh'), (b_hh, 'b_hh'), (act, 'act'),
                 (c, 'c'), (h, 'h')):
        _chk(t, 'lstm_step_fwd.' + n)
    _lib.call('gx_lstm_step_fwd', _p(gx), _p(h_prev), _p(c_prev), _p(w_hh), _p(b_hh), B, H4 // 4, _p(act), _p(c),
              _p(h), _stream())


def lstm_step_bwd(g_h, dgates_next, w_hh, act, c, c_prev, dc_next, dgates, dc_prev):
    B, H4 = act.shape
    for t, n in ((g_h, 'g_h'), (dgates_next, 'dgates_next'), (act, 'act'), (c, 'c'), (c_prev, 'c_prev'),
                 (dc_next, 'dc_next'), (dgates, 'dgates'), (dc_prev, 'dc_prev')):
        _chk(t, 'lstm_step_bwd.' + n)
    _lib.call('gx_lstm_step_bwd', _p(g_h), _p(dgates_next), _p(w_hh), _p(act), _p(c), _p(c_prev), _p(dc_next), B,
              H4 // 4, _p(dgates), _p(dc_prev), _stream())


LSTM_SEQ = os.environ.get('GENESIS_LSTM_SEQ', '0') == '1'
_LSTM_BAR = {}


def _lstm_bar(device, which):
    key = (device.index, torch.cuda.current_stream(device).cuda_stream, which)
    t = _LSTM_BAR.get(key)
    if t is None:
        t = _LSTM_BAR[key] = torch.zeros(_lib.query('gx_lstm_seq_ws_bytes') // 4, dtype=torch.int32, device=device)
    return t


def lstm_seq_steps(B, H):
    return lstm_seq_capacity(B, H) if LSTM_SEQ else 0


def lstm_seq_capacity(B, H):
    return _lib.query('gx_lstm_seq_max_steps', B, H)


def lstm_seq_fwd(gx3, w_hh, b_hh, act, c, h):
    T, B, H4 = gx3.shape
    for t, n in ((gx3, 'gx'), (w_hh, 'w_hh'), (b_hh, 'b_hh'), (act, 'act'), (c, 'c'), (h, 'h')):
        _chk(t, 'lstm_seq_fwd.' + n)
    _lib.call('gx_lstm_seq_fwd', _p(gx3), _p(w_hh), _p(b_hh), T, B, H4 // 4, _p(act), _p(c), _p(h),
              _p(_lstm_bar(gx3.device, 0)), _stream())


def lstm_seq_bwd(g_h, w_hh, act, c, dgates, dc2):
    T, B, H4 = act.shape
    for t, n in ((g_h, 'g_h'), (w_hh, 'w_hh'), (act, 'act'), (c, 'c'), (dgates, 'dgates'), (dc2, 'dc2')):
        _chk(t, 'lstm_seq_bwd.' + n)
    _lib.call('gx_lstm_seq_bwd', _p(g_h), _p(w_hh), _p(act), _p(c), T, B, H4 // 4, _p(dgates), _p(dc2),
              _p(_lstm_bar(act.device, 1)), _stream())


def conv1x1_gn_fwd(y_pre, mean, rstd, gamma, beta, groups, w, bias, gate=None, addend=None):
    _chk(y_pre, 'conv1x1_gn.y'); _chk(mean, 'conv1x1_gn.mean'); _chk(rstd, 'conv1x1_gn.rstd')
    _chk(gamma, 'conv1x1_gn.gamma'); _chk(beta, 'conv1x1_gn.beta'); _chk(w, 'conv1x1_gn.w'); _chk(bias, 'conv1x1_gn.bias')
    _chk(gate, 'conv1x1_gn.gate'); _chk(addend, 'conv1x1_gn.addend')
    N, Cin, H, W = y_pre.shape
    Cout = w.shape[0]
    out = torch.empty(N, Cout, H, W, dtype=F32, device=y_pre.device)
    _lib.call('gx_conv1x1_gn_fwd', _p(y_pre), _p(mean), _p(rstd), _p(gamma), _p(beta), groups, _p(w), _p(bias),
              _p(gate), _p(addend), N, Cin, Cout, H, W, _p(out), _stream())
    return out


def conv1x1_gn_wgrad(y_pre, mean, rstd, gamma, beta, groups, g_out, w=None, bias=None, gate=None, out=None):
    _chk(y_pre, 'conv1x1_gn_wgrad.y'); _chk(g_out, 'conv1x1_gn_wgrad.g')
    N, Cin, H, W = y_pre.shape
    Cout = g_out.shape[1]
    o = out or (None, None, None)
    dw = o[0] if o[0] is not None else torch.empty(Cout, Cin, dtype=F32, device=y_pre.device)
    db = o[1] if o[1] is not None else torch.empty(Cout, dtype=F32, device=y_pre.device)
    dgate = (o[2] if o[2] is not None else torch.empty((), dtype=F32, device=y_pre.device)) if gate is not None else None
    _chk(dw, 'conv1x1_gn_wgrad.dw'); _chk(db, 'conv1x1_gn_wgrad.db'); _chk(dgate, 'conv1x1_gn_wgrad.dgate')
    assert dw.numel() == Cout * Cin and db.numel() == Cout
    nb = _lib.query('gx_conv1x1_gn_wgrad_ws_bytes', N, Cin, Cout, H, W)
    ws = _ws(nb, y_pre.device)
    _lib.call('gx_conv1x1_gn_wgrad', _p(y_pre), _p(mean), _p(rstd), _p(gamma), _p(beta), groups, _p(g_out), _p(w),
              _p(bias), _p(gate), N, Cin, Cout, H, W, _p(dw), _p(db), _p(dgate), _p(ws), nb, _stream())
    return dw, db, dgate


def conv1x1_gn_bwd_fused(y, gamma, beta, mean, rstd, groups, g_out, w, bias, gate=None, want_dbias=False,
                         out_gn=None, out_conv=None):
    N, C, H, W = y.shape
    Cout = int(g_out.shape[1])
    if not _lib.query('gx_gn_relu_bwd_proj_fuses_wgrad', C, H, W, groups, Cout):
        return None
    wpart = torch.empty(N, Cout, C, dtype=F32, device=y.device)
    bpart = torch.empty(N, Cout, dtype=F32, device=y.device)
    dy, dgamma, dbeta, dbias = gn_relu_bwd_proj(y, gamma, beta, mean, rstd, groups, g_out, w, want_dbias, out_gn, gate,
                                                parts=(wpart, bpart))
    o = out_conv or (None, None, None)
    dw = o[0] if o[0] is not None else torch.empty(Cout, C, dtype=F32, device=y.device)
    db = o[1] if o[1] is not None else torch.empty(Cout, dtype=F32, device=y.device)
    dgate = (o[2] if o[2] is not None else torch.empty((), dtype=F32, device=y.device)) if gate is not None else None
    _chk(dw, 'conv1x1_gn_bwd.dw'); _chk(db, 'conv1x1_gn_bwd.db'); _chk(dgate, 'conv1x1_gn_bwd.dgate')
    assert dw.numel() == Cout * C and db.numel() == Cout
    nb = _lib.query('gx_conv1x1_gn_wgrad_finish_ws_bytes', C, Cout)
    ws = _ws(nb, y.device)
    _lib.call('gx_conv1x1_gn_wgrad_finish', _p(wpart), _p(bpart), N, C, Cout, _p(w), _p(bias), _p(gate), _p(dw), _p(db),
              _p(dgate), _p(ws), nb, _stream())
    return dy, (dgamma, dbeta, dbias), (dw, db, dgate)


def gn_relu_bwd_proj(y, gamma, beta, mean, rstd, groups, g_out, w, want_dbias=False, out=None, gate=None,
                     parts=(None, None)):
    _chk(y, 'gn_bwd_proj.y'); _chk(g_out, 'gn_bwd_proj.g'); _chk(w, 'gn_bwd_proj.w')
    N, C, H, W = y.shape
    dy = torch.empty_like(y)
    o = out or (None, None, None)
    dgamma = o[0] if o[0] is not None else torch.empty(C, dtype=F32, device=y.device)
    dbeta = o[1] if o[1] is not None else torch.empty(C, dtype=F32, device=y.device)
    dbias = (o[2] if o[2] is not None else torch.empty(C, dtype=F32, device=y.device)) if want_dbias else None
    nb = _lib.query('gx_gn_relu_bwd_proj_ws_bytes', N, C, H, W, groups, int(g_out.shape[1]))
    ws = _ws(nb, y.device)
    direct = o[0] is not None and o[1] is not None and (not want_dbias or o[2] is not None)
    tap = _tap_begin(y.device, H * W, y.numel())
    with _deferring(direct, ws):
        _lib.call('gx_gn_relu_bwd_proj', _p(y), _p(gamma), _p(beta), _p(mean), _p(rstd), N, C, H, W, groups,
                  _p(g_out), int(g_out.shape[1]), _p(w), _p(gate), _p(dy), _p(dgamma), _p(dbeta), _p(dbias),
# ... 61 lines not shown
```

### include/genesis_hip.h

```cpp
#ifndef GENESIS_HIP_H
#define GENESIS_HIP_H
#include <stddef.h>
#include <stdint.h>

#ifdef __cplusplus
extern "C" {
#endif

typedef void* gx_stream_t;

#define GX_OK 0
#define GX_EINVAL (-1)
#define GX_ELAUNCH (-2)
#define GX_EDATA (-3)

const char* gx_last_error(void);
int gx_version(void);

size_t gx_conv3x3_ws_bytes(int N, int Cin, int Cout, int H, int W);
int gx_conv3x3_fwd(const float* x, const float* w, float* y, int N, int Cin, int Cout, int H, int W,
                   void* ws, size_t ws_bytes, gx_stream_t stream);
int gx_conv3x3_dgrad(const float* dy, const float* w, float* dx, int N, int Cin, int Cout, int H, int W,
                     void* ws, size_t ws_bytes, gx_stream_t stream);
int gx_conv3x3_dgrad_parts(const float* dy, const float* w, float* dx, int N, int Cin, int Cout, int H, int W, void* ws,
// ... 146 lines not shown
int gx_profile_enable(int on);
int gx_profile_num_kernels(void);
const char* gx_profile_kernel_name(int kid);
int gx_profile_collect(double* total_ms, double* launches, double* flops, double* bytes);

int gx_conv3x3_bias_act_fwd(const float* x, const float* w, const float* bias, int act, float* y, int N, int Cin,
                            int Cout, int H, int W, void* ws, size_t ws_bytes, gx_stream_t stream);
size_t gx_bias_act_bwd_ws_bytes(int N, int C);
int gx_bias_act_bwd(const float* out, const float* g, int N, int C, int H, int W, int act, float* dy, float* dbias,
                    void* ws, size_t ws_bytes, gx_stream_t stream);
int gx_conv3x3_dgrad_act_supported(int N, int Cin, int Cout, int H, int W);
size_t gx_conv3x3_dgrad_act_ws_bytes(int N, int Cin, int Cout, int H, int W);
int gx_conv3x3_dgrad_act(const float* dy, const float* w, const float* xout, int act, float* dxa, float* dbias, int N,
                         int Cin, int Cout, int H, int W, void* ws, size_t ws_bytes, gx_stream_t stream);
int gx_conv3x3_wgrad_quad_supported(int N, int C, int H, int W);
size_t gx_conv3x3_wgrad_quad_ws_bytes(int N, int C, int H, int W);
int gx_conv3x3_wgrad_quad(const float* x, const float* dy, float* dw, int N, int C, int H, int W, void* ws, size_t ws_bytes,
                          gx_stream_t stream);
size_t gx_conv3x3_wgrad_quad_bias_ws_bytes(int N, int C, int H, int W);
int gx_conv3x3_wgrad_quad_bias(const float* x, const float* dy, float* dw, float* dbias, int N, int C, int H, int W, void* ws,
                               size_t ws_bytes, gx_stream_t stream);
int gx_conv5x5s1_supported(int N, int K, int M, int H, int W);
size_t gx_conv5x5s1_ws_bytes(int N, int K, int M, int H, int W);
int gx_conv5x5s1(const float* in, const float* w, float* out, int N, int K, int M, int H, int W, int flip, void* ws,
                 size_t ws_bytes, gx_stream_t stream);
int gx_conv5x5_wgrad_supported(int N, int CA, int CB, int H, int W);
size_t gx_conv5x5_wgrad_ws_bytes(int N, int CA, int CB, int H, int W);
int gx_conv5x5_wgrad(const float* a, const float* b, float* dw, int N, int CA, int CB, int H, int W, void* ws,
                     size_t ws_bytes, gx_stream_t stream);

int gx_conv3x3s2_dgrad_small(const float* dy, const float* w, float* dx, int N, int Cin, int Cout, int H, int W, int cin_n,
                             gx_stream_t stream);
int gx_conv3x3s2_dgrad_small_ex(const float* dy, const float* w, float* dx, int N, int Cin, int Cout, int H, int W, int cin_n,
                                int dx_channels, gx_stream_t stream);
int gx_mask_image_stack(const float* mask, const float* x, float* out, int K, int B, int C, int H, int W, gx_stream_t stream);
size_t gx_conv3x3s2_wgrad_small_ws_bytes(int N, int Cin, int Cout, int H, int W);
int gx_conv3x3s2_wgrad_small(const float* x, const float* dy, float* dw, int N, int Cin, int Cout, int H, int W, void* ws,
                             size_t ws_bytes, gx_stream_t stream);
int gx_conv2d_direct_fwd(const float* x, const float* w, const float* bias, int act, float* y, int N, int Cin,
                         int Cout, int H, int W, int k, int stride, int pad, gx_stream_t stream);
size_t gx_conv2d_direct_fwd_ws_bytes(int N, int Cin, int Cout, int H, int W, int k, int stride, int pad);
int gx_conv2d_direct_fwd_ws(const float* x, const float* w, const float* bias, int act, float* y, int N, int Cin,
                            int Cout, int H, int W, int k, int stride, int pad, void* ws, size_t ws_bytes,
                            gx_stream_t stream);
int gx_conv2d_direct_dgrad(const float* dy, const float* w, float* dx, int N, int Cin, int Cout, int H, int W, int k,
                           int stride, int pad, gx_stream_t stream);
size_t gx_conv2d_direct_wgrad_ws_bytes(int N, int Cin, int Cout, int H, int W, int k, int stride, int pad);
int gx_conv2d_direct_wgrad(const float* x, const float* dy, float* dw, int N, int Cin, int Cout, int H, int W, int k,
                           int stride, int pad, void* ws, size_t ws_bytes, gx_stream_t stream);
int gx_mixture_w_fwd(const float* x, const float* dec, const float* log_w, int dec_ch, int B, int H, int W, int K,
                     float pixel_std1, float pixel_std2, int pixel_bound, float* recon, float* x_r, float* err,
                     void* ws, size_t ws_bytes, gx_stream_t stream);
int gx_mixture_w_bwd(const float* x, const float* dec, const float* log_w, const float* g_err, int dec_ch, int B,
                     int H, int W, int K, float pixel_std1, float pixel_std2, int pixel_bound, float* ddec,
                     float* dlog_w, gx_stream_t stream);

size_t gx_gated_stats_floats(int norm, int N, int C);
int gx_gated_norm_fwd(const float* y, const float* bias, int norm, const float* gamma_h, const float* beta_h,
                      const float* gamma_g, const float* beta_g, int N, int C, int H, int W, float eps, float* out,
                      float* stats, gx_stream_t stream);
int gx_bn_running_update(const float* stats, int C, double m, float eps, float momentum, float* rm_h, float* rv_h, float* rm_g,
                         float* rv_g, long long* nbt_h, long long* nbt_g, gx_stream_t stream);
int gx_gated_bn_running(float* rm_h, float* rv_h, float* rm_g, float* rv_g, long long* nbt_h, long long* nbt_g, float momentum);
size_t gx_gated_norm_bwd_ws_bytes(int norm, int N, int C);
int gx_gated_norm_bwd(const float* y, const float* bias, int norm, const float* gamma_h, const float* beta_h,
                      const float* gamma_g, const float* beta_g, const float* stats, const float* dout, int N, int C,
                      int H, int W, float* dy, float* dgamma_h, float* dbeta_h, float* dgamma_g, float* dbeta_g,
                      float* dbias, void* ws, size_t ws_bytes, gx_stream_t stream);

size_t gx_gated_bn_sums_ws_bytes(int N, int C);
int gx_gated_bn_local_sums(const float* y, const float* bias, int N, int C, int H, int W, double* sums, void* ws,
                           size_t ws_bytes, gx_stream_t stream);
int gx_gated_bn_apply(const float* y, const float* bias, const double* sums, double m, const float* gamma_h,
                      const float* beta_h, const float* gamma_g, const float* beta_g, int N, int C, int H, int W, float eps,
                      float* out, float* stats, gx_stream_t stream);
int gx_gated_bn_bwd_local_sums(const float* y, const float* bias, const float* gamma_h, const float* beta_h,
                               const float* gamma_g, const float* beta_g, const float* stats, const float* dout, int N, int C,
                               int H, int W, float* sums, float* dgamma_h, float* dbeta_h, float* dgamma_g, float* dbeta_g,
                               float* dbias, void* ws, size_t ws_bytes, gx_stream_t stream);
int gx_gated_bn_bwd_apply(const float* y, const float* bias, const float* gamma_h, const float* beta_h, const float* gamma_g,
                          const float* beta_g, const float* stats, const float* dout, const float* sums, double m, int N, int C,
                          int H, int W, float* dy, gx_stream_t stream);

int gx_sbp_scan_fwd(const float* logits, const float* log_s0, int T, size_t P, int last_scope, float* log_m,
                    float* log_s, gx_stream_t stream);
int gx_sbp_scan_bwd(const float* logits, const float* g_log_m, const float* g_log_s, int T, size_t P, int last_scope,
                    float* g_logits, float* g_log_s0, gx_stream_t stream);
int gx_categorical_kl_fwd(const float* log_m, const float* log_m_r, int K, int B, int HW, float* kl,
                          gx_stream_t stream);
int gx_categorical_kl_bwd(const float* log_m, const float* log_m_r, const float* g_kl, int K, int B, int HW,
                          float* g_log_m, float* g_log_m_r, gx_stream_t stream);
int gx_logsoftmax_k_fwd(const float* dec, int K, int B, int HW, int C, float* log_m_r, gx_stream_t stream);
int gx_logsoftmax_k_bwd(const float* log_m_r, const float* g, int K, int B, int HW, int C, float* g_dec,
                        gx_stream_t stream);

int gx_broadcast_concat(const float* z, const float* coords, float* out, int N, int D, int d, gx_stream_t stream);
int gx_bcast_deconv5x5s2_pack(const float* w, const float* b, const float* coords, int D, int Cout, int d, float* wz,
                              float* bias, gx_stream_t stream);
int gx_bcast_deconv5x5s2_unpack(const float* dwz, const float* dbias, const float* coords, int D, int Cout, int d,
                                float* dw, float* db, gx_stream_t stream);
int gx_bcast_conv3x3_fwd(const float* z, const float* w, const float* bias, const float* rowc, const float* colc,
                         int act, float* out, int N, int L, int Co, int d, gx_stream_t stream);
size_t gx_bcast_conv3x3_bwd_ws_bytes(int N, int Co);
int gx_bcast_conv3x3_bwd(const float* y, const float* g, const float* z, const float* w, const float* rowc,
                         const float* colc, int act, int N, int L, int Co, int d, float* dz, float* dw, float* db,
                         void* ws, size_t ws_bytes, gx_stream_t stream);

int gx_latent_posterior_fwd(const float* zh, const float* eps, int B, int K, int D, float* z, float* mu,
                            float* sigma, float* log_q, gx_stream_t stream);
int gx_latent_posterior_bwd(const float* zh, const float* eps, const float* gz, const float* gmu,
                            const float* gsigma, const float* glogq, int B, int K, int D, float* dzh,
                            gx_stream_t stream);
int gx_latent_posterior_fwd_ex(const float* zh, const float* eps, int B, int K, int D, float* z, float* mu,
                               float* sigma, float* log_q, float* z2, int ldz2, gx_stream_t stream);
int gx_latent_posterior_bwd_ex(const float* zh, const float* eps, const float* gz, const float* gmu,
                               const float* gsigma, const float* glogq, const float* gz2, int ldgz2, int B, int K,
                               int D, float* dzh, gx_stream_t stream);
int gx_latent_prior_logp_fwd(const float* z, const float* lin, const float* log_q, int B, int K, int D,
                             float* out, gx_stream_t stream);
int gx_latent_prior_logp_bwd(const float* z, const float* lin, const float* g_out, int kl_mode, int B, int K,
                             int D, float* dz, float* dlin, gx_stream_t stream);
int gx_latent_prior_logp_fwd_ex(const float* z, const float* lin, const float* log_q, int B, int K, int D, int all_slots,
                                float* out, gx_stream_t stream);
int gx_latent_prior_logp_bwd_ex(const float* z, const float* lin, const float* g_out, int kl_mode, int B, int K,
                                int D, int all_slots, float* dz, float* dlin, gx_stream_t stream);
int gx_latent_prior_sample(const float* lin, const float* eps, int B, int D, float* z, gx_stream_t stream);
int gx_latent_prior_sample_ex(const float* lin, const float* eps, int B, int D, int tanh_mu, float* z,
                              gx_stream_t stream);

int gx_elbo_fwd(const float* err, const float* kl, const float* beta, int B, int R, float* out, float* tail,
                float* loss, gx_stream_t stream);
int gx_elbo_fwd_grads(const float* err, const float* kl, const float* beta, int B, int R, float* out, float* tail,
                      float* loss, float* d_err, float* d_kl, gx_stream_t stream);
int gx_elbo_bwd(const float* g_loss, const float* beta, int B, int R, float* d_err, float* d_kl,
                gx_stream_t stream);

int gx_pooled_head_fwd(const float* lin, const float* msum, const float* fbias, const float* gamma,
                       const float* beta, float eps, int R, int C, float* y, float* stats, gx_stream_t stream);
size_t gx_pooled_head_bwd_ws_bytes(int R, int C);
int gx_pooled_head_bwd(const float* lin, const float* msum, const float* fbias, const float* gamma,
                       const float* stats, const float* g, int R, int C, float* dlin, float* dmsum, float* dfbias,
                       float* dgamma, float* dbeta, void* ws, size_t ws_bytes, gx_stream_t stream);

int gx_linear_fwd(const float* x, const float* w, const float* b, int act, float* y, int M, int N, int K,
                  gx_stream_t stream);
int gx_linear_bwd(const float* x, const float* w, const float* y, const float* g, int act, float* dx, float* dw,
                  float* db, int M, int N, int K, gx_stream_t stream);
int gx_linear_fwd_ld(const float* x, int ldx, const float* w, const float* b, int act, float* y, int ldy, int M,
                     int N, int K, gx_stream_t stream);
int gx_linear_bwd_ex(const float* x, int ldx, const float* w, const float* y, const float* g, int ldg, int act,
                     float* dx, int lddx, int dx_accumulate, float* dw, float* db, float* db2, int M, int N, int K,
                     gx_stream_t stream);

int gx_matmul_nn_fwd(const float* x, const float* w, float* y, int M, int N, int K, gx_stream_t stream);
size_t gx_matmul_nn_bwd_ws_bytes(int M, int N, int K);
int gx_matmul_nn_bwd(const float* x, const float* w, const float* g, float* dx, float* dw, int M, int N, int K,
                     void* ws, size_t ws_bytes, gx_stream_t stream);

int gx_lstm_step_fwd(const float* gx, const float* h_prev, const float* c_prev, const float* w_hh,
                     const float* b_hh, int B, int H, float* act, float* c, float* h, gx_stream_t stream);
int gx_lstm_step_bwd(const float* g_h, const float* dgates_next, const float* w_hh, const float* act,
                     const float* c, const float* c_prev, const float* dc_next, int B, int H, float* dgates,
                     float* dc_prev, gx_stream_t stream);
int gx_lstm_seq_max_steps(int B, int H);
size_t gx_lstm_seq_ws_bytes(void);
int gx_lstm_seq_fwd(const float* gx, const float* w_hh, const float* b_hh, int T, int B, int H, float* act, float* c,
                    float* h, void* bar, gx_stream_t stream);
int gx_lstm_seq_bwd(const float* g_h, const float* w_hh, const float* act, const float* c, int T, int B, int H,
                    float* dgates, float* dc2, void* bar, gx_stream_t stream);

int gx_weight_cache_create(void);
int gx_weight_cache_record(int id, int on);
int gx_weight_cache_size(int id);
int gx_weight_cache_refresh(int id, gx_stream_t stream);
int gx_weight_cache_release(void);
int gx_weight_cache_activate(int id);
int gx_weight_cache_destroy(int id);

int gx_ctx_create(void);
int gx_ctx_make_current(int id);
int gx_ctx_current(void);
int gx_ctx_destroy(int id);

int gx_defer_enable(int on);
int gx_defer_pending(void);
int gx_defer_flush(gx_stream_t stream);

int gx_conv3x3_fwd_parts(const float* x, const float* w, float* y, int N, int Cin, int Cout, int H, int W, void* ws,
                         size_t ws_bytes, const float** parts, int* nsplit, size_t* split_stride, gx_stream_t stream);
int gx_deconv5x5s2_fwd_parts(const float* x, const float* w, float* y, int N, int Cin, int Cout, int Hin, int Win,
                             void* ws, size_t ws_bytes, const float** parts, int* nsplit, size_t* split_stride,
                             gx_stream_t stream);
int gx_gn_relu_fwd_parts(const float* parts, int nsplit, size_t split_stride, const float* conv_bias, float* y_sum,
                         const float* gamma, const float* beta, int N, int C, int H, int W, int groups, float eps,
                         float* dst0, int dst0_ctot, int dst0_c0, int dst0_mode, float* dst1, int dst1_ctot,
                         int dst1_c0, int dst1_mode, float* mean, float* rstd, gx_stream_t stream);

int gx_label_contingency(const long long* segA, const long long* segB, int B, int HW, int KA, int KB, int* counts,
                         gx_stream_t stream);

#define GX_FID_MAXPOOL_S2 0
#define GX_FID_MAXPOOL_S1P1 1
#define GX_FID_AVGPOOL_S1P1 2
#define GX_FID_GLOBAL_AVGPOOL 3
int gx_fid_preprocess(const float* x, float* y, int B, int H, int W, int quantise, gx_stream_t stream);
int gx_fid_conv_bias_relu(const float* x, int B, int H, int W, int Cin, const float* w, const float* bias, int kh, int kw,
                          int stride, int ph, int pw, float* d0, int d0_ctot, int d0_c0, int n0, float* d1, int d1_ctot,
                          int d1_c0, int n1, float* d2, int d2_ctot, int d2_c0, int n2, gx_stream_t stream);
int gx_fid_pool(const float* x, int B, int H, int W, int C, int mode, float* y, int y_ctot, int y_c0, gx_stream_t stream);
int gx_fid_moments(const float* feats, int B, int D, double* sum, double* sumsq, gx_stream_t stream);

int gx_u8hwc_to_f32chw(const unsigned char* src, float* dst, int B, int Hs, int Ws, int C, int H, int W,
                       gx_stream_t stream);

#define GX_RESAMPLE_NEAREST 0
#define GX_RESAMPLE_PIL_BILINEAR 1
#define GX_LABEL_U8 0
#define GX_LABEL_I32 1
#define GX_LABEL_I64 2
int gx_pil_bilinear_ksize(int in, int out);
int gx_pil_bilinear_coeffs(int in, int out, int ksize, int* bounds, int* weights);
int gx_u8hwc_resample_f32chw(const unsigned char* src, float* dst, int B, int Hs, int Ws, int C, int top, int left, int Hc,
                             int Wc, int H, int W, int mode, const int* hbounds, const int* hweights, int hksize,
                             const int* vbounds, const int* vweights, int vksize, gx_stream_t stream);
int gx_labels_crop_nearest(const void* src, int dtype, long long* dst, int B, int Hs, int Ws, int top, int left, int Hc, int Wc,
                           int H, int W, gx_stream_t stream);

#define GX_ROWS_U8 0
#define GX_ROWS_F32 1
#define GX_LABEL_F32 3
#define GX_LABEL_F64 4
int gx_rows_gather_f32chw(const void* src, int dtype, long long N, const long long* idx, long long idx_len, long long first,
                          float* dst, int B, int Hs, int Ws, int C, int H, int W, gx_stream_t stream);
int gx_rows_gather_labels(const void* src, int dtype, long long N, const long long* idx, long long idx_len, long long first,
                          long long* dst, int B, int Hs, int Ws, int H, int W, gx_stream_t stream);
int gx_sprites_compose(const unsigned char* sprites, int S, const int* first, const int* count, const unsigned char* colours,
                       float* img, unsigned char* mask, int n, gx_stream_t stream);

unsigned int gx_crc32c(const void* data, size_t n);
unsigned int gx_crc32c_masked(const void* data, size_t n);
int gx_tfrecord_scan(const unsigned char* buf, size_t n, int verify_crc, long long first_index, int max_records,
                     long long* offsets, long long* lengths, int* num_records, size_t* consumed);
int gx_tfexample_find_bytes_list(const unsigned char* rec, size_t n, const char* name, long long* offset, long long* length);
int gx_bytes_list_unpack(const unsigned char* payload, size_t n, unsigned char* dst, size_t expected);
int gx_entity_masks_to_labels(const unsigned char* masks, long long* dst, int B, int E, int Hs, int Ws, long long entity_stride,
                              long long pixel_stride, int background_entities, int top, int left, int Hc, int Wc, int H, int W,
                              gx_stream_t stream);

int gx_bytes_list_index(const unsigned char* payload, size_t n, int max_values, long long* offsets, long long* lengths, int* count);
int gx_jpeg_info(const unsigned char* data, size_t len, int* info);
int gx_jpeg_entropy_decode(const unsigned char* data, size_t len, short* coef, size_t coef_capacity, unsigned short* qtab,
                           int* info);
int gx_jpeg_decode_f32chw(const short* coef, const unsigned short* qtab, float* dst_f32, unsigned char* dst_u8, int B, int H, int W,
                          int sampling, int S_h, int S_w, gx_stream_t stream);

#define GX_PNG_PLANE_BYTE 0
#define GX_PNG_PLANE_SHAPESTACKS_REF 1
#define GX_PNG_PLANE_INDEX 2
int gx_png_info(const unsigned char* data, size_t len, int* info);
int gx_png_inflate(const unsigned char* data, size_t len, unsigned char* dst, size_t dst_capacity, int* info);
int gx_png_unfilter(const unsigned char* filtered, unsigned char* dst_u8, unsigned char* dst_plane0, int plane_rule, int B, int H,
                    int W, int C, gx_stream_t stream);

size_t gx_allreduce_unique_id_bytes(void);
int gx_allreduce_unique_id(void* id, size_t id_bytes);
int gx_allreduce_init(const void* id, size_t id_bytes, int rank, int world, void** comm);
int gx_allreduce_run(void* comm, float* buf, size_t count, gx_stream_t stream);
int gx_allreduce_destroy(void* comm);

int gx_mfma_fp32_probe(int wgs, int iters, int mode, float* scratch, double* flops, gx_stream_t stream);

#ifdef __cplusplus
}
#endif
#endif
```

Before: 12290.

## Fuse slot posterior head into single forward and batched backward kernels

Adds a fused slot-head path that runs the pooled feature linear, layer norm, two dense layers and the posterior sampling in one forward launch. The backward pass also runs as one row kernel plus a single multi-job dense launch for all weight gradients. The aim is to remove the many small kernel launches and intermediate round trips in this small per-slot MLP. In exchange it adds a large new kernel file with an eligibility check and falls back to the old path otherwise. The shared dense tile and latent row helpers are moved into headers so both paths can use them.

```diff
diff --git a/genesis_amd/build.py b/genesis_amd/build.py
--- a/genesis_amd/build.py
+++ b/genesis_amd/build.py
@@ -6,7 +6,7 @@
 HERE = osp.dirname(osp.abspath(__file__))
 CSRC = osp.join(HERE, 'csrc')
 LIB = osp.join(HERE, 'libgenesis_hip.so')
-SOURCES = ['gx_api.cpp', 'gx_comm.cpp', 'gx_conv.hip', 'gx_norm.hip', 'gx_attention.hip', 'gx_slots.hip', 'gx_optim.hip', 'gx_misc.hip', 'gx_gated.hip', 'gx_latent.hip', 'gx_dense.hip', 'gx_igemm.hip', 'gx_metrics.hip', 'gx_feed.hip', 'gx_wino.hip', 'gx_kq.hip', 'gx_bcast.hip', 'gx_sbp.hip', 'gx_wgq.hip', 'gx_wstrip.hip', 'gx_fid.hip', 'gx_tfrecord.cpp', 'gx_jpeg.cpp', 'gx_jpeg.hip', 'gx_png.cpp', 'gx_png.hip', 'gx_multid.hip']
+SOURCES = ['gx_api.cpp', 'gx_comm.cpp', 'gx_conv.hip', 'gx_norm.hip', 'gx_attention.hip', 'gx_slots.hip', 'gx_optim.hip', 'gx_misc.hip', 'gx_gated.hip', 'gx_latent.hip', 'gx_dense.hip', 'gx_slot_head.hip', 'gx_igemm.hip', 'gx_metrics.hip', 'gx_feed.hip', 'gx_wino.hip', 'gx_kq.hip', 'gx_bcast.hip', 'gx_sbp.hip', 'gx_wgq.hip', 'gx_wstrip.hip', 'gx_fid.hip', 'gx_tfrecord.cpp', 'gx_jpeg.cpp', 'gx_jpeg.hip', 'gx_png.cpp', 'gx_png.hip', 'gx_multid.hip']
 HIPCC = os.environ.get('HIPCC', '/opt/rocm/bin/hipcc')
 FLAGS = ['--offload-arch=gfx950', '-O3', '-std=c++17', '-fPIC', '-Wno-unused-value',
          '-Wno-pass-failed']
@@ -14,7 +14,8 @@
 
 def _deps():
     d = [osp.join(CSRC, s) for s in SOURCES if osp.exists(osp.join(CSRC, s))]
-    d += [osp.join(CSRC, 'gx_common.h'), osp.join(osp.dirname(HERE), 'include', 'genesis_hip.h'), osp.join(HERE, 'pk_peephole.py')]
+    d += [osp.join(CSRC, h) for h in ('gx_common.h', 'gx_dense_tile.h', 'gx_latent_rows.h')]
+    d += [osp.join(osp.dirname(HERE), 'include', 'genesis_hip.h'), osp.join(HERE, 'pk_peephole.py')]
     return d
 
 
diff --git a/genesis_amd/csrc/gx_dense.hip b/genesis_amd/csrc/gx_dense.hip
--- a/genesis_amd/csrc/gx_dense.hip
+++ b/genesis_amd/csrc/gx_dense.hip
@@ -1,110 +1,8 @@
 #include "gx_common.h"
+#include "gx_dense_tile.h"
 
 namespace {
 
-__device__ __forceinline__ float mask_factor(float m, bool elu) { return m > 0.f ? 1.f : (elu ? m + 1.f : 0.f); }
-
-template <bool A_KC, bool B_KC, bool MASK, bool ROWSUM>
-__device__ __forceinline__ void
-dense_tile(float (*part)[256], float (*rpart)[16], int bx, int by, const float* __restrict__ a, int lda,
-           const float* __restrict__ mask, const float* __restrict__ b, int ldb, const float* __restrict__ bias,
-           int act, float* __restrict__ c, int ldc, int I, int J, int Kc, float* __restrict__ rs, int vec_a,
-           int vec_b, float* __restrict__ rs2 = nullptr) {
-    const int lane = threadIdx.x & 63, wave = threadIdx.x >> 6, nw = blockDim.x >> 6;
-    const int idx = lane & 15, kq = lane >> 4;
-    const int i0 = by * 16, j0 = bx * 16;
-    const bool elu_mask = (act & 4) != 0;
-    const bool acc_rs = (act & 8) != 0;
-    act &= 3;
-    const int ai = i0 + idx, bj = j0 + idx;
-    const bool a_ok = ai < I, b_ok = bj < J;
-    f32x4 acc = {0.f, 0.f, 0.f, 0.f};
-    float rsum = 0.f;
-#pragma unroll 2
-    for (int k16 = wave * 16; k16 < Kc; k16 += nw * 16) {
-        const int kb = k16 + 4 * kq;
-        float av[4], bv[4];
-        if (A_KC) {
-            if (vec_a) {
-                f32x4 t = {0.f, 0.f, 0.f, 0.f}, m = {1.f, 1.f, 1.f, 1.f};
-                if (a_ok && kb < Kc) {
-                    t = *reinterpret_cast<const f32x4*>(a + (size_t)ai * lda + kb);
-                    if (MASK) m = *reinterpret_cast<const f32x4*>(mask + (size_t)ai * lda + kb);
-                }
-#pragma unroll
-                for (int jj = 0; jj < 4; ++jj) av[jj] = MASK ? t[jj] * mask_factor(m[jj], elu_mask) : t[jj];
-            } else {
-#pragma unroll
-                for (int jj = 0; jj < 4; ++jj) {
-                    float t = 0.f;
-                    if (a_ok && kb + jj < Kc) {
-                        t = a[(size_t)ai * lda + kb + jj];
-                        if (MASK) t *= mask_factor(mask[(size_t)ai * lda + kb + jj], elu_mask);
-                    }
-                    av[jj] = t;
-                }
-            }
-        } else {
-#pragma unroll
-            for (int jj = 0; jj < 4; ++jj) {
-                float t = 0.f;
-                if (a_ok && kb + jj < Kc) {
-                    t = a[(size_t)(kb + jj) * lda + ai];
-                    if (MASK) t *= mask_factor(mask[(size_t)(kb + jj) * lda + ai], elu_mask);
-                }
-                av[jj] = t;
-            }
-        }
-        if (B_KC) {
-            if (vec_b) {
-                f32x4 t = {0.f, 0.f, 0.f, 0.f};
-                if (b_ok && kb < Kc) t = *reinterpret_cast<const f32x4*>(b + (size_t)bj * ldb + kb);
-#pragma unroll
-                for (int jj = 0; jj < 4; ++jj) bv[jj] = t[jj];
-            } else {
-#pragma unroll
-                for (int jj = 0; jj < 4; ++jj)
-                    bv[jj] = (b_ok && kb + jj < Kc) ? b[(size_t)bj * ldb + kb + jj] : 0.f;
-            }
-        } else {
-#pragma unroll
-            for (int jj = 0; jj < 4; ++jj)
-                bv[jj] = (b_ok && kb + jj < Kc) ? b[(size_t)(kb + jj) * ldb + bj] : 0.f;
-        }
-#pragma unroll
-        for (int jj = 0; jj < 4; ++jj) {
-            acc = __builtin_amdgcn_mfma_f32_16x16x4f32(av[jj], bv[jj], acc, 0, 0, 0);
-            if (ROWSUM) rsum += av[jj];
-        }
-    }
-#pragma unroll
-    for (int r = 0; r < 4; ++r) part[wave][(kq * 4 + r) * 16 + idx] = acc[r];
-    if (ROWSUM) {
-        rsum += __shfl_xor(rsum, 16, 64);
-        rsum += __shfl_xor(rsum, 32, 64);
-        if (kq == 0) rpart[wave][idx] = rsum;
-    }
-    __syncthreads();
-    if (threadIdx.x < 256) {
-        const int t = threadIdx.x;
-        float s = part[0][t];
-        for (int w = 1; w < nw; ++w) s += part[w][t];
-        const int ci = i0 + (t >> 4), cj = j0 + (t & 15);
-        if (ci < I && cj < J) {
-            if (bias) s += bias[cj];
-            if (act == 1) s = s > 0.f ? s : 0.f;
-            if (act == 2) s += c[(size_t)ci * ldc + cj];
-            if (act == 3) s = s > 0.f ? s : expm1f(s);
-            c[(size_t)ci * ldc + cj] = s;
-        }
-    }
-    if (ROWSUM && bx == 0 && threadIdx.x < 16 && i0 + (int)threadIdx.x < I) {
-        float s = rpart[0][threadIdx.x];
-        for (int w = 1; w < nw; ++w) s += rpart[w][threadIdx.x];
-        if (acc_rs) { rs[i0 + threadIdx.x] += s; if (rs2) rs2[i0 + threadIdx.x] += s; }
-        else { rs[i0 + threadIdx.x] = s; if (rs2) rs2[i0 + threadIdx.x] = s; }
-    }
-}
 
 template <bool A_KC, bool B_KC, bool MASK, bool ROWSUM>
 __global__ void __launch_bounds__(1024)
@@ -451,9 +349,6 @@
     return tiles < 128 ? tiles : 128;
 }
 
-inline bool aligned16(const void* p) { return (reinterpret_cast<uintptr_t>(p) & 15) == 0; }
-inline int dense_threads(int Kc) { return Kc >= 1024 ? 1024 : 256; }
-
 }
 
 extern "C" {
diff --git a/genesis_amd/csrc/gx_dense_tile.h b/genesis_amd/csrc/gx_dense_tile.h
--- /dev/null
+++ b/genesis_amd/csrc/gx_dense_tile.h
@@ -0,0 +1,137 @@
+#pragma once
+#include "gx_common.h"
+
+namespace {
+
+__device__ __forceinline__ float mask_factor(float m, bool elu) { return m > 0.f ? 1.f : (elu ? m + 1.f : 0.f); }
+
+template <bool A_KC, bool B_KC, bool MASK, bool ROWSUM, int NT = 1>
+__device__ __forceinline__ void
+dense_tile_g(float (*part)[256], float (*rpart)[16], int gtid, int wave, int nw, int bx, int by,
+             const float* __restrict__ a, int lda, const float* __restrict__ mask, const float* __restrict__ b, int ldb,
+             const float* __restrict__ bias, int act, float* __restrict__ c, int ldc, int I, int J, int Kc,
+             float* __restrict__ rs, int vec_a, int vec_b, float* __restrict__ rs2 = nullptr, int bxs = 0, int ps = 0) {
+    const int lane = gtid & 63;
+    const int idx = lane & 15, kq = lane >> 4;
+    const int i0 = by * 16;
+    const bool elu_mask = (act & 4) != 0;
+    const bool acc_rs = (act & 8) != 0;
+    act &= 3;
+    const int ai = i0 + idx;
+    const bool a_ok = ai < I;
+    f32x4 acc[NT];
+#pragma unroll
+    for (int t = 0; t < NT; ++t) { acc[t][0] = 0.f; acc[t][1] = 0.f; acc[t][2] = 0.f; acc[t][3] = 0.f; }
+    float rsum = 0.f;
+#pragma unroll 2
+    for (int k16 = wave * 16; k16 < Kc; k16 += nw * 16) {
+        const int kb = k16 + 4 * kq;
+        float av[4], bv[NT][4];
+        if (A_KC) {
+            if (vec_a) {
+                f32x4 t = {0.f, 0.f, 0.f, 0.f}, m = {1.f, 1.f, 1.f, 1.f};
+                if (a_ok && kb < Kc) {
+                    t = *reinterpret_cast<const f32x4*>(a + (size_t)ai * lda + kb);
+                    if (MASK) m = *reinterpret_cast<const f32x4*>(mask + (size_t)ai * lda + kb);
+                }
+#pragma unroll
+                for (int jj = 0; jj < 4; ++jj) av[jj] = MASK ? t[jj] * mask_factor(m[jj], elu_mask) : t[jj];
+            } else {
+#pragma unroll
+                for (int jj = 0; jj < 4; ++jj) {
+                    float t = 0.f;
+                    if (a_ok && kb + jj < Kc) {
+                        t = a[(size_t)ai * lda + kb + jj];
+                        if (MASK) t *= mask_factor(mask[(size_t)ai * lda + kb + jj], elu_mask);
+                    }
+                    av[jj] = t;
+                }
+            }
+        } else {
+#pragma unroll
+            for (int jj = 0; jj < 4; ++jj) {
+                float t = 0.f;
+                if (a_ok && kb + jj < Kc) {
+                    t = a[(size_t)(kb + jj) * lda + ai];
+                    if (MASK) t *= mask_factor(mask[(size_t)(kb + jj) * lda + ai], elu_mask);
+                }
+                av[jj] = t;
+            }
+        }
+#pragma unroll
+        for (int t = 0; t < NT; ++t) {
+            const int bj = (bx + t * bxs) * 16 + idx;
+            const bool b_ok = bj < J;
+            if (B_KC) {
+                if (vec_b) {
+                    f32x4 v = {0.f, 0.f, 0.f, 0.f};
+                    if (b_ok && kb < Kc) v = *reinterpret_cast<const f32x4*>(b + (size_t)bj * ldb + kb);
+#pragma unroll
+                    for (int jj = 0; jj < 4; ++jj) bv[t][jj] = v[jj];
+                } else {
+#pragma unroll
+                    for (int jj = 0; jj < 4; ++jj)
+                        bv[t][jj] = (b_ok && kb + jj < Kc) ? b[(size_t)bj * ldb + kb + jj] : 0.f;
+                }
+            } else {
+#pragma unroll
+                for (int jj = 0; jj < 4; ++jj)
+                    bv[t][jj] = (b_ok && kb + jj < Kc) ? b[(size_t)(kb + jj) * ldb + bj] : 0.f;
+            }
+        }
+#pragma unroll
+        for (int jj = 0; jj < 4; ++jj) {
+#pragma unroll
+            for (int t = 0; t < NT; ++t)
+                acc[t] = __builtin_amdgcn_mfma_f32_16x16x4f32(av[jj], bv[t][jj], acc[t], 0, 0, 0);
+            if (ROWSUM) rsum += av[jj];
+        }
+    }
+#pragma unroll
+    for (int t = 0; t < NT; ++t)
+#pragma unroll
+        for (int r = 0; r < 4; ++r) part[t * ps + wave][(kq * 4 + r) * 16 + idx] = acc[t][r];
+    if (ROWSUM) {
+        rsum += __shfl_xor(rsum, 16, 64);
+        rsum += __shfl_xor(rsum, 32, 64);
+        if (kq == 0) rpart[wave][idx] = rsum;
+    }
+    __syncthreads();
+    if (gtid < 256) {
+        const int t = gtid;
+#pragma unroll
+        for (int u = 0; u < NT; ++u) {
+            float s = part[u * ps][t];
+            for (int w = 1; w < nw; ++w) s += part[u * ps + w][t];
+            const int ci = i0 + (t >> 4), cj = (bx + u * bxs) * 16 + (t & 15);
+            if (ci < I && cj < J) {
+                if (bias) s += bias[cj];
+                if (act == 1) s = s > 0.f ? s : 0.f;
+                if (act == 2) s += c[(size_t)ci * ldc + cj];
+                if (act == 3) s = s > 0.f ? s : expm1f(s);
+                c[(size_t)ci * ldc + cj] = s;
+            }
+        }
+    }
+    if (ROWSUM && bx == 0 && gtid < 16 && i0 + gtid < I) {
+        float s = rpart[0][gtid];
+        for (int w = 1; w < nw; ++w) s += rpart[w][gtid];
+        if (acc_rs) { rs[i0 + gtid] += s; if (rs2) rs2[i0 + gtid] += s; }
+        else { rs[i0 + gtid] = s; if (rs2) rs2[i0 + gtid] = s; }
+    }
+}
+
+template <bool A_KC, bool B_KC, bool MASK, bool ROWSUM>
+__device__ __forceinline__ void
+dense_tile(float (*part)[256], float (*rpart)[16], int bx, int by, const float* __restrict__ a, int lda,
+           const float* __restrict__ mask, const float* __restrict__ b, int ldb, const float* __restrict__ bias,
+           int act, float* __restrict__ c, int ldc, int I, int J, int Kc, float* __restrict__ rs, int vec_a,
+           int vec_b, float* __restrict__ rs2 = nullptr) {
+    dense_tile_g<A_KC, B_KC, MASK, ROWSUM>(part, rpart, (int)threadIdx.x, (int)(threadIdx.x >> 6), (int)(blockDim.x >> 6), bx, by,
+                                           a, lda, mask, b, ldb, bias, act, c, ldc, I, J, Kc, rs, vec_a, vec_b, rs2);
+}
+
+inline bool aligned16(const void* p) { return (reinterpret_cast<uintptr_t>(p) & 15) == 0; }
+inline int dense_threads(int Kc) { return Kc >= 1024 ? 1024 : 256; }
+
+}
diff --git a/genesis_amd/csrc/gx_latent.hip b/genesis_amd/csrc/gx_latent.hip
--- a/genesis_amd/csrc/gx_latent.hip
+++ b/genesis_amd/csrc/gx_latent.hip
@@ -1,18 +1,7 @@
 #include "gx_common.h"
+#include "gx_latent_rows.h"
 
 namespace {
-
-constexpr float kHalfLog2Pi = 0.91893853320467274178f;
-
-__device__ __forceinline__ float softplus_t(float x) {
-    return x > 20.f ? x : log1pf(expf(x));
-}
-__device__ __forceinline__ float softplus_grad_t(float x) {
-    if (x > 20.f) return 1.f;
-    const float e = expf(x);
-    return e / (e + 1.f);
-}
-__device__ __forceinline__ float sigmoid_t(float x) { return 1.f / (1.f + expf(-x)); }
 
 __global__ void __launch_bounds__(256)
 posterior_fwd_kernel(const float* __restrict__ zh, const float* __restrict__ eps, int B, int K, int D,
@@ -20,24 +9,7 @@
                      float* __restrict__ log_q, float* __restrict__ z2, int ldz2) {
     const int row = blockIdx.x * (blockDim.x >> 6) + (threadIdx.x >> 6);
     if (row >= K * B) return;
-    const int lane = threadIdx.x & 63;
-    const int k = row / B, b = row - k * B;
-    const float* zr = zh + ((size_t)b * K + k) * 2 * D;
-    double acc = 0.0;
-    for (int d = lane; d < D; d += 64) {
-        const float mu = zr[d];
-        const float sg = softplus_t(zr[D + d] + 0.5f) + 1e-8f;
-        const float zz = mu + sg * eps[(size_t)row * D + d];
-        const float t = zz - mu;
-        const float lp = -(t * t) / (2.f * (sg * sg)) - logf(sg) - kHalfLog2Pi;
-        z[(size_t)row * D + d] = zz;
-        if (z2) z2[(size_t)row * ldz2 + d] = zz;
-        mu_o[(size_t)row * D + d] = mu;
-        sigma_o[(size_t)row * D + d] = sg;
-        acc += (double)lp;
-    }
-    acc = gx_wave_sum_d(acc);
-    if (lane == 0) log_q[row] = (float)acc;
+    posterior_fwd_row(row, threadIdx.x & 63, zh, eps, B, K, D, z, mu_o, sigma_o, log_q, z2, ldz2);
 }
 
 __global__ void __launch_bounds__(256)
@@ -47,26 +19,7 @@
                      const float* __restrict__ gz2, int ldgz2) {
     const int row = blockIdx.x * (blockDim.x >> 6) + (threadIdx.x >> 6);
     if (row >= K * B) return;
-    const int lane = threadIdx.x & 63;
-    const int k = row / B, b = row - k * B;
-    const float* zr = zh + ((size_t)b * K + k) * 2 * D;
-    float* dr = dzh + ((size_t)b * K + k) * 2 * D;
-    const float gl = glogq ? glogq[row] : 0.f;
-    for (int d = lane; d < D; d += 64) {
-        const size_t i = (size_t)row * D + d;
-        const float mu = zr[d];
-        const float raw = zr[D + d] + 0.5f;
-        const float sg = softplus_t(raw) + 1e-8f;
-        const float e = eps[i];
-        const float zz = mu + sg * e;
-        const float t = zz - mu;
-        const float var = sg * sg;
-        const float dz = (gz ? gz[i] : 0.f) + (gz2 ? gz2[(size_t)row * ldgz2 + d] : 0.f) + gl * (-t / var);
-        const float dmu = dz + gl * (t / var) + (gmu ? gmu[i] : 0.f);
-        const float dsg = dz * e + gl * ((t * t) / (var * sg) - 1.f / sg) + (gsigma ? gsigma[i] : 0.f);
-        dr[d] = dmu;
-        dr[D + d] = dsg * softplus_grad_t(raw);
-    }
+    posterior_bwd_row(row, threadIdx.x & 63, zh, eps, gz, gmu, gsigma, glogq, B, K, D, dzh, gz2, ldgz2);
 }
 
 __global__ void __launch_bounds__(256)
@@ -178,24 +131,7 @@
                        float* __restrict__ stats ) {
     const int row = blockIdx.x * (blockDim.x >> 6) + (threadIdx.x >> 6);
     if (row >= R) return;
-    const int lane = threadIdx.x & 63;
-    const float m = msum[row];
-    const float den = m + 1e-5f;
-    double s1 = 0.0, s2 = 0.0;
-    for (int j = lane; j < C; j += 64) {
-        const float o = (lin[(size_t)row * C + j] + m * fbias[j]) / den;
-        s1 += (double)o; s2 += (double)o * o;
-    }
-    s1 = gx_wave_sum_d(s1); s2 = gx_wave_sum_d(s2);
-    const double mean = s1 / C;
-    double var = s2 / C - mean * mean;
-    if (var < 0.0) var = 0.0;
-    const float meanf = (float)mean, rstd = (float)(1.0 / sqrt(var + (double)eps));
-    for (int j = lane; j < C; j += 64) {
-        const float o = (lin[(size_t)row * C + j] + m * fbias[j]) / den;
-        y[(size_t)row * C + j] = (o - meanf) * rstd * gamma[j] + beta[j];
-    }
-    if (lane == 0) { stats[2 * row] = meanf; stats[2 * row + 1] = rstd; }
+    pooled_head_fwd_row(row, threadIdx.x & 63, lin, msum, fbias, gamma, beta, eps, C, y, stats);
 }
 
 __global__ void __launch_bounds__(256)
@@ -205,52 +141,14 @@
                        float* __restrict__ dlin, float* __restrict__ dmsum, float* __restrict__ cols) {
     const int row = blockIdx.x * (blockDim.x >> 6) + (threadIdx.x >> 6);
     if (row >= R) return;
-    const int lane = threadIdx.x & 63;
-    const float m = msum[row];
-    const float den = m + 1e-5f;
-    const float meanf = stats[2 * row], rstd = stats[2 * row + 1];
-    double a = 0.0, b = 0.0;
-    for (int j = lane; j < C; j += 64) {
-        const float o = (lin[(size_t)row * C + j] + m * fbias[j]) / den;
-        const float xh = (o - meanf) * rstd;
-        const float dxh = g[(size_t)row * C + j] * gamma[j];
-        a += (double)dxh; b += (double)dxh * xh;
-    }
-    a = gx_wave_sum_d(a); b = gx_wave_sum_d(b);
-    const float k1 = (float)(a / C), k2 = (float)(b / C);
-    double dm = 0.0;
-    for (int j = lane; j < C; j += 64) {
-        const float num = lin[(size_t)row * C + j] + m * fbias[j];
-        const float o = num / den;
-        const float xh = (o - meanf) * rstd;
-        const float gv = g[(size_t)row * C + j];
-        const float dobj = rstd * (gv * gamma[j] - k1 - xh * k2);
-        dlin[(size_t)row * C + j] = dobj / den;
-        dm += (double)dobj * ((double)fbias[j] / den - (double)num / ((double)den * den));
-        float* cr = cols + (size_t)row * 3 * C;
-        cr[j] = gv * xh; cr[C + j] = gv; cr[2 * C + j] = dobj * (m / den);
-    }
-    dm = gx_wave_sum_d(dm);
-    if (lane == 0) dmsum[row] = (float)dm;
+    pooled_head_bwd_row(row, threadIdx.x & 63, lin, msum, fbias, gamma, stats, g, C, dlin, dmsum, cols);
 }
 
 __global__ void __launch_bounds__(256)
 pooled_head_cols_kernel(const float* __restrict__ cols, int R, int C, float* __restrict__ dgamma,
                         float* __restrict__ dbeta, float* __restrict__ dfbias) {
     __shared__ double red[8][32];
-    const int cl = threadIdx.x & 31, rg = threadIdx.x >> 5;
-    const int i = blockIdx.x * 32 + cl;
-    double s = 0.0;
-    if (i < 3 * C)
-        for (int r = rg; r < R; r += 8) s += (double)cols[(size_t)r * 3 * C + i];
-    red[rg][cl] = s;
-    __syncthreads();
-    if (rg == 0 && i < 3 * C) {
-        double t = red[0][cl];
-        for (int q = 1; q < 8; ++q) t += red[q][cl];
-        const int which = i / C, j = i - which * C;
-        (which == 0 ? dgamma : (which == 1 ? dbeta : dfbias))[j] = (float)t;
-    }
+    pooled_head_cols_block(red, threadIdx.x, blockIdx.x, cols, R, C, dgamma, dbeta, dfbias);
 }
 
 int check_bkd(const char* name, int B, int K, int D) {
diff --git a/genesis_amd/csrc/gx_latent_rows.h b/genesis_amd/csrc/gx_latent_rows.h
--- /dev/null
+++ b/genesis_amd/csrc/gx_latent_rows.h
@@ -0,0 +1,141 @@
+#pragma once
+#include "gx_common.h"
+
+namespace {
+
+constexpr float kHalfLog2Pi = 0.91893853320467274178f;
+
+__device__ __forceinline__ float softplus_t(float x) {
+    return x > 20.f ? x : log1pf(expf(x));
+}
+__device__ __forceinline__ float softplus_grad_t(float x) {
+    if (x > 20.f) return 1.f;
+    const float e = expf(x);
+    return e / (e + 1.f);
+}
+__device__ __forceinline__ float sigmoid_t(float x) { return 1.f / (1.f + expf(-x)); }
+
+__device__ __forceinline__ void
+posterior_fwd_row(int row, int lane, const float* __restrict__ zh, const float* __restrict__ eps, int B, int K, int D,
+                  float* __restrict__ z, float* __restrict__ mu_o, float* __restrict__ sigma_o,
+                  float* __restrict__ log_q, float* __restrict__ z2, int ldz2) {
+    const int k = row / B, b = row - k * B;
+    const float* zr = zh + ((size_t)b * K + k) * 2 * D;
+    double acc = 0.0;
+    for (int d = lane; d < D; d += 64) {
+        const float mu = zr[d];
+        const float sg = softplus_t(zr[D + d] + 0.5f) + 1e-8f;
+        const float zz = mu + sg * eps[(size_t)row * D + d];
+        const float t = zz - mu;
+        const float lp = -(t * t) / (2.f * (sg * sg)) - logf(sg) - kHalfLog2Pi;
+        z[(size_t)row * D + d] = zz;
+        if (z2) z2[(size_t)row * ldz2 + d] = zz;
+        mu_o[(size_t)row * D + d] = mu;
+        sigma_o[(size_t)row * D + d] = sg;
+        acc += (double)lp;
+    }
+    acc = gx_wave_sum_d(acc);
+    if (lane == 0) log_q[row] = (float)acc;
+}
+
+__device__ __forceinline__ void
+posterior_bwd_row(int row, int lane, const float* __restrict__ zh, const float* __restrict__ eps,
+                  const float* __restrict__ gz, const float* __restrict__ gmu, const float* __restrict__ gsigma,
+                  const float* __restrict__ glogq, int B, int K, int D, float* __restrict__ dzh,
+                  const float* __restrict__ gz2, int ldgz2) {
+    const int k = row / B, b = row - k * B;
+    const float* zr = zh + ((size_t)b * K + k) * 2 * D;
+    float* dr = dzh + ((size_t)b * K + k) * 2 * D;
+    const float gl = glogq ? glogq[row] : 0.f;
+    for (int d = lane; d < D; d += 64) {
+        const size_t i = (size_t)row * D + d;
+        const float mu = zr[d];
+        const float raw = zr[D + d] + 0.5f;
+        const float sg = softplus_t(raw) + 1e-8f;
+        const float e = eps[i];
+        const float zz = mu + sg * e;
+        const float t = zz - mu;
+        const float var = sg * sg;
+        const float dz = (gz ? gz[i] : 0.f) + (gz2 ? gz2[(size_t)row * ldgz2 + d] : 0.f) + gl * (-t / var);
+        const float dmu = dz + gl * (t / var) + (gmu ? gmu[i] : 0.f);
+        const float dsg = dz * e + gl * ((t * t) / (var * sg) - 1.f / sg) + (gsigma ? gsigma[i] : 0.f);
+        dr[d] = dmu;
+        dr[D + d] = dsg * softplus_grad_t(raw);
+    }
+}
+
+__device__ __forceinline__ void
+pooled_head_fwd_row(int row, int lane, const float* __restrict__ lin, const float* __restrict__ msum,
+                    const float* __restrict__ fbias, const float* __restrict__ gamma, const float* __restrict__ beta,
+                    float eps, int C, float* __restrict__ y, float* __restrict__ stats ) {
+    const float m = msum[row];
+    const float den = m + 1e-5f;
+    double s1 = 0.0, s2 = 0.0;
+    for (int j = lane; j < C; j += 64) {
+        const float o = (lin[(size_t)row * C + j] + m * fbias[j]) / den;
+        s1 += (double)o; s2 += (double)o * o;
+    }
+    s1 = gx_wave_sum_d(s1); s2 = gx_wave_sum_d(s2);
+    const double mean = s1 / C;
+    double var = s2 / C - mean * mean;
+    if (var < 0.0) var = 0.0;
+    const float meanf = (float)mean, rstd = (float)(1.0 / sqrt(var + (double)eps));
+    for (int j = lane; j < C; j += 64) {
+        const float o = (lin[(size_t)row * C + j] + m * fbias[j]) / den;
+        y[(size_t)row * C + j] = (o - meanf) * rstd * gamma[j] + beta[j];
+    }
+    if (lane == 0) { stats[2 * row] = meanf; stats[2 * row + 1] = rstd; }
+}
+
+__device__ __forceinline__ void
+pooled_head_bwd_row(int row, int lane, const float* __restrict__ lin, const float* __restrict__ msum,
+                    const float* __restrict__ fbias, const float* __restrict__ gamma, const float* __restrict__ stats,
+                    const float* __restrict__ g, int C, float* __restrict__ dlin, float* __restrict__ dmsum,
+                    float* __restrict__ cols) {
+    const float m = msum[row];
+    const float den = m + 1e-5f;
+    const float meanf = stats[2 * row], rstd = stats[2 * row + 1];
+    double a = 0.0, b = 0.0;
+    for (int j = lane; j < C; j += 64) {
+        const float o = (lin[(size_t)row * C + j] + m * fbias[j]) / den;
+        const float xh = (o - meanf) * rstd;
+        const float dxh = g[(size_t)row * C + j] * gamma[j];
+        a += (double)dxh; b += (double)dxh * xh;
+    }
+    a = gx_wave_sum_d(a); b = gx_wave_sum_d(b);
+    const float k1 = (float)(a / C), k2 = (float)(b / C);
+    double dm = 0.0;
+    for (int j = lane; j < C; j += 64) {
+        const float num = lin[(size_t)row * C + j] + m * fbias[j];
+        const float o = num / den;
+        const float xh = (o - meanf) * rstd;
+        const float gv = g[(size_t)row * C + j];
+        const float dobj = rstd * (gv * gamma[j] - k1 - xh * k2);
+        dlin[(size_t)row * C + j] = dobj / den;
+        dm += (double)dobj * ((double)fbias[j] / den - (double)num / ((double)den * den));
+        float* cr = cols + (size_t)row * 3 * C;
+        cr[j] = gv * xh; cr[C + j] = gv; cr[2 * C + j] = dobj * (m / den);
+    }
+    dm = gx_wave_sum_d(dm);
+    if (lane == 0) dmsum[row] = (float)dm;
+}
+
+__device__ __forceinline__ void
+pooled_head_cols_block(double (*red)[32], int tid, int block, const float* __restrict__ cols, int R, int C,
+                       float* __restrict__ dgamma, float* __restrict__ dbeta, float* __restrict__ dfbias) {
+    const int cl = tid & 31, rg = tid >> 5;
+    const int i = block * 32 + cl;
+    double s = 0.0;
+    if (i < 3 * C)
+        for (int r = rg; r < R; r += 8) s += (double)cols[(size_t)r * 3 * C + i];
+    red[rg][cl] = s;
+    __syncthreads();
+    if (rg == 0 && i < 3 * C) {
+        double t = red[0][cl];
+        for (int q = 1; q < 8; ++q) t += red[q][cl];
+        const int which = i / C, j = i - which * C;
+        (which == 0 ? dgamma : (which == 1 ? dbeta : dfbias))[j] = (float)t;
+    }
+}
+
+}
diff --git a/genesis_amd/csrc/gx_slot_head.hip b/genesis_amd/csrc/gx_slot_head.hip
--- /dev/null
+++ b/genesis_amd/csrc/gx_slot_head.hip
@@ -0,0 +1,210 @@
+#include "gx_common.h"
+#include "gx_dense_tile.h"
+#include "gx_latent_rows.h"
+#include "../../include/genesis_hip.h"
+
+namespace {
+
+constexpr int kDmMaxJobs = 8;
+
+struct DmTable {
+    gx_dense_job j[kDmMaxJobs];
+    int start[kDmMaxJobs + 1];
+    int n;
+};
+
+__device__ __forceinline__ void stage_sync() {
+    __threadfence_block();
+    __syncthreads();
+}
+
+__global__ void __launch_bounds__(256)
+dense_multi_kernel(const DmTable tab) {
+    __shared__ float part[4][256];
+    __shared__ float rpart[4][16];
+    __shared__ double red[8][32];
+    int jb = 0;
+    while (jb + 1 < tab.n && (int)blockIdx.x >= tab.start[jb + 1]) ++jb;
+    const gx_dense_job& q = tab.j[jb];
+    const int local = (int)blockIdx.x - tab.start[jb];
+    if (q.kind == GX_DJ_COLS) {
+        pooled_head_cols_block(red, threadIdx.x, local, q.a, q.I, q.J, q.c, q.rs, q.rs2);
+        return;
+    }
+    const int nx = (q.J + 15) >> 4;
+    const int bx = local % nx, by = local / nx;
+#define GX_DM(MASK, ROWSUM)                                                                                             \
+    dense_tile<false, false, MASK, ROWSUM>(part, rpart, bx, by, q.a, q.lda, q.mask, q.b, q.ldb, nullptr, q.act, q.c, q.ldc, \
+                                           q.I, q.J, q.Kc, q.rs, 0, 0, q.rs2)
+    if (q.mask) { if (q.rs) GX_DM(true, true); else GX_DM(true, false); }
+    else        { if (q.rs) GX_DM(false, true); else GX_DM(false, false); }
+#undef GX_DM
+}
+
+struct SlotHeadFwd {
+    const float *S, *msum, *wf, *fbias, *gamma, *beta, *w1, *b1, *w3, *b3, *noise;
+    float *lin, *stats, *y, *h1, *zh, *z, *mu, *sigma, *log_q;
+    float eps;
+    int B, K, Cin, C, N1, D;
+};
+
+#define GX_ROW_GEMM(A_KC, B_KC, MASK, J, ...)                                                                       \
+    for (int jt0 = 0; jt0 < ((J) + 15) / 16; jt0 += 8) {                                                            \
+        dense_tile_g<A_KC, B_KC, MASK, false, 2>(gp, gr, gtid, gw, 4, jt0 + grp, by, __VA_ARGS__, nullptr, 4, 16);  \
+        stage_sync();                                                                                               \
+    }
+
+__global__ void __launch_bounds__(1024)
+slot_head_fwd_kernel(const SlotHeadFwd p) {
+    __shared__ float part[32][256];
+    __shared__ float rpart[16][16];
+    const int wave = threadIdx.x >> 6, lane = threadIdx.x & 63;
+    const int grp = wave >> 2, gw = wave & 3, gtid = threadIdx.x & 255;
+    float (*gp)[256] = part + grp * 4;
+    float (*gr)[16] = rpart + grp * 4;
+    const int by = blockIdx.x, R = p.B * p.K, row = by * 16 + wave;
+    GX_ROW_GEMM(true, true, false, p.C, p.S, p.Cin, nullptr, p.wf, p.Cin, nullptr, 0, p.lin, p.C, R, p.C, p.Cin, nullptr, 1, 1)
+    if (row < R) pooled_head_fwd_row(row, lane, p.lin, p.msum, p.fbias, p.gamma, p.beta, p.eps, p.C, p.y, p.stats);
+    stage_sync();
+    GX_ROW_GEMM(true, true, false, p.N1, p.y, p.C, nullptr, p.w1, p.C, p.b1, 1, p.h1, p.N1, R, p.N1, p.C, nullptr, 1, 1)
+    GX_ROW_GEMM(true, true, false, 2 * p.D, p.h1, p.N1, nullptr, p.w3, p.N1, p.b3, 0, p.zh, 2 * p.D, R, 2 * p.D, p.N1, nullptr, 1, 1)
+    if (row < R) {
+        const int b = row / p.K, k = row - b * p.K;
+        posterior_fwd_row(k * p.B + b, lane, p.zh, p.noise, p.B, p.K, p.D, p.z, p.mu, p.sigma, p.log_q, nullptr, 0);
+    }
+}
+
+struct SlotHeadBwd {
+    const float *zh, *noise, *gz, *gz2, *gmu, *gsigma, *glogq, *w3, *h1, *w1, *lin, *msum, *fbias, *gamma, *stats, *wf;
+    float *dzh, *dh1, *dy, *dlin, *dmsum, *cols, *dS;
+    int B, K, Cin, C, N1, D;
+};
+
+__global__ void __launch_bounds__(1024)
+slot_head_bwd_kernel(const SlotHeadBwd p) {
+    __shared__ float part[32][256];
+    __shared__ float rpart[16][16];
+    const int wave = threadIdx.x >> 6, lane = threadIdx.x & 63;
+    const int grp = wave >> 2, gw = wave & 3, gtid = threadIdx.x & 255;
+    float (*gp)[256] = part + grp * 4;
+    float (*gr)[16] = rpart + grp * 4;
+    const int by = blockIdx.x, R = p.B * p.K, row = by * 16 + wave;
+    if (row < R) {
+        const int b = row / p.K, k = row - b * p.K;
+        posterior_bwd_row(k * p.B + b, lane, p.zh, p.noise, p.gz, p.gmu, p.gsigma, p.glogq, p.B, p.K, p.D, p.dzh, p.gz2, p.D);
+    }
+    stage_sync();
+    GX_ROW_GEMM(true, false, false, p.N1, p.dzh, 2 * p.D, nullptr, p.w3, p.N1, nullptr, 0, p.dh1, p.N1, R, p.N1, 2 * p.D, nullptr, 1, 0)
+    GX_ROW_GEMM(true, false, true, p.C, p.dh1, p.N1, p.h1, p.w1, p.C, nullptr, 0, p.dy, p.C, R, p.C, p.N1, nullptr, 1, 0)
+    if (row < R) pooled_head_bwd_row(row, lane, p.lin, p.msum, p.fbias, p.gamma, p.stats, p.dy, p.C, p.dlin, p.dmsum, p.cols);
+    stage_sync();
+    GX_ROW_GEMM(true, false, false, p.Cin, p.dlin, p.C, nullptr, p.wf, p.Cin, nullptr, 0, p.dS, p.Cin, R, p.Cin, p.C, nullptr, 1, 0)
+}
+
+#undef GX_ROW_GEMM
+
+inline bool dim_ok(int n) { return n > 0 && n < 1024 && n % 4 == 0; }
+
+}
+
+extern "C" {
+
+int gx_dense_multi(const gx_dense_job* jobs, int njobs, gx_stream_t stream) {
+    GX_CHECK_ARG(jobs, "gx_dense_multi: null job table");
+    GX_CHECK_ARG(njobs > 0 && njobs <= kDmMaxJobs, "gx_dense_multi: %d jobs (1..%d)", njobs, kDmMaxJobs);
+    DmTable tab;
+    tab.n = njobs;
+    int blocks = 0;
+    double flops = 0.0, bytes = 0.0;
+    for (int i = 0; i < njobs; ++i) {
+        const gx_dense_job& q = jobs[i];
+        GX_CHECK_ARG(q.kind == GX_DJ_DW || q.kind == GX_DJ_COLS, "gx_dense_multi: job %d: unknown kind %d", i, q.kind);
+        GX_CHECK_ARG(q.I > 0 && q.J > 0, "gx_dense_multi: job %d: bad sizes (%d,%d)", i, q.I, q.J);
+        tab.j[i] = q;
+        tab.start[i] = blocks;
+        if (q.kind == GX_DJ_COLS) {
+            GX_CHECK_ARG(q.a && q.c && q.rs && q.rs2, "gx_dense_multi: job %d: null pointer", i);
+            blocks += gx_ceil_div(3 * q.J, 32);
+            bytes += 4.0 * 3.0 * q.I * q.J;
+            continue;
+        }
+        GX_CHECK_ARG(q.a && q.b && q.c, "gx_dense_multi: job %d: null pointer", i);
+        GX_CHECK_ARG(q.Kc > 0 && q.Kc < 1024, "gx_dense_multi: job %d: contraction length %d (1..1023)", i, q.Kc);
+        GX_CHECK_ARG(q.act == 0 || q.act == 10, "gx_dense_multi: job %d: act is 0 (write) or 10 (add to c, rs, rs2), got %d", i, q.act);
+        GX_CHECK_ARG(q.rs || !q.rs2, "gx_dense_multi: job %d: rs2 is a second copy of rs", i);
+        GX_CHECK_ARG(q.lda >= q.I && q.ldb >= q.J && q.ldc >= q.J, "gx_dense_multi: job %d: a row stride is shorter than its rows", i);
+        blocks += gx_ceil_div(q.I, 16) * gx_ceil_div(q.J, 16);
+        flops += 2.0 * q.I * q.J * q.Kc;
+        bytes += 4.0 * ((double)q.I * q.Kc + (double)q.J * q.Kc + (double)q.I * q.J);
+    }
+    tab.start[njobs] = blocks;
+    hipStream_t s = (hipStream_t)stream;
+    {
+        GxProf pf(KID_DENSE, s, flops, bytes);
+        hipLaunchKernelGGL(dense_multi_kernel, dim3(blocks), dim3(256), 0, s, tab);
+    }
+    GX_CHECK_LAUNCH("gx_dense_multi");
+    return GX_OK;
+}
+
+int gx_slot_head_eligible(int B, int K, int Cin, int C, int N1, int D) {
+    if (B <= 0 || K <= 0 || (long long)B * K >= 1024) return 0;
+    return dim_ok(Cin) && dim_ok(C) && dim_ok(N1) && dim_ok(D) && 2 * D < 1024;
+}
+
+int gx_slot_head_fwd(const float* S, const float* msum, const float* wf, const float* fbias, const float* gamma,
+                     const float* beta, float eps, const float* w1, const float* b1, const float* w3, const float* b3,
+                     const float* noise, int B, int K, int Cin, int C, int N1, int D, float* lin, float* stats, float* y,
+                     float* h1, float* zh, float* z, float* mu, float* sigma, float* log_q, gx_stream_t stream) {
+    GX_CHECK_ARG(S && msum && wf && fbias && gamma && beta && w1 && b1 && w3 && b3 && noise && lin && stats && y && h1 && zh &&
+                 z && mu && sigma && log_q, "gx_slot_head_fwd: null pointer");
+    GX_CHECK_ARG(gx_slot_head_eligible(B, K, Cin, C, N1, D),
+                 "gx_slot_head_fwd: sizes B=%d K=%d Cin=%d C=%d N1=%d D=%d are not eligible (gx_slot_head_eligible)", B, K, Cin, C,
+                 N1, D);
+    GX_CHECK_ARG(aligned16(S) && aligned16(wf) && aligned16(w1) && aligned16(w3) && aligned16(y) && aligned16(h1),
+                 "gx_slot_head_fwd: 16-byte alignment");
+    const SlotHeadFwd p = {S, msum, wf, fbias, gamma, beta, w1, b1, w3, b3, noise, lin, stats, y, h1, zh, z, mu, sigma, log_q,
+                           eps, B, K, Cin, C, N1, D};
+    hipStream_t s = (hipStream_t)stream;
+    const double R = (double)B * K;
+    {
+        GxProf pf(KID_LATENT, s, 2.0 * R * ((double)C * Cin + (double)N1 * C + 2.0 * D * N1),
+                  4.0 * (R * (Cin + 3.0 * C + 2.0 * N1 + 8.0 * D) + (double)C * Cin + (double)N1 * C + 2.0 * D * N1));
+        hipLaunchKernelGGL(slot_head_fwd_kernel, dim3(gx_ceil_div(B * K, 16)), dim3(1024), 0, s, p);
+    }
+    GX_CHECK_LAUNCH("gx_slot_head_fwd");
+    return GX_OK;
+}
+
+size_t gx_slot_head_bwd_ws_bytes(int B, int K, int C) {
+    if (B <= 0 || K <= 0 || C <= 0) return 0;
+    return (size_t)B * K * 3 * C * sizeof(float);
+}
+
+int gx_slot_head_bwd_rows(const float* zh, const float* noise, const float* gz, const float* gz2, const float* gmu,
+                          const float* gsigma, const float* glogq, const float* w3, const float* h1, const float* w1,
+                          const float* lin, const float* msum, const float* fbias, const float* gamma, const float* stats,
+                          const float* wf, int B, int K, int Cin, int C, int N1, int D, float* dzh, float* dh1, float* dy,
+                          float* dlin, float* dmsum, float* dS, void* ws, size_t ws_bytes, gx_stream_t stream) {
+    GX_CHECK_ARG(zh && noise && w3 && h1 && w1 && lin && msum && fbias && gamma && stats && wf && dzh && dh1 && dy && dlin &&
+                 dmsum && dS && ws, "gx_slot_head_bwd_rows: null pointer");
+    GX_CHECK_ARG(gx_slot_head_eligible(B, K, Cin, C, N1, D),
+                 "gx_slot_head_bwd_rows: sizes B=%d K=%d Cin=%d C=%d N1=%d D=%d are not eligible (gx_slot_head_eligible)", B, K,
+                 Cin, C, N1, D);
+    GX_CHECK_ARG(ws_bytes >= gx_slot_head_bwd_ws_bytes(B, K, C), "gx_slot_head_bwd_rows: workspace too small");
+    GX_CHECK_ARG(aligned16(dzh) && aligned16(dh1) && aligned16(h1) && aligned16(dlin),
+                 "gx_slot_head_bwd_rows: 16-byte alignment");
+    const SlotHeadBwd p = {zh, noise, gz, gz2, gmu, gsigma, glogq, w3, h1, w1, lin, msum, fbias, gamma, stats, wf,
+                           dzh, dh1, dy, dlin, dmsum, (float*)ws, dS, B, K, Cin, C, N1, D};
+    hipStream_t s = (hipStream_t)stream;
+    const double R = (double)B * K;
+    {
+        GxProf pf(KID_LATENT, s, 2.0 * R * ((double)C * Cin + (double)N1 * C + 2.0 * D * N1),
+                  4.0 * (R * (Cin + 8.0 * C + 3.0 * N1 + 10.0 * D) + (double)C * Cin + (double)N1 * C + 2.0 * D * N1));
+        hipLaunchKernelGGL(slot_head_bwd_kernel, dim3(gx_ceil_div(B * K, 16)), dim3(1024), 0, s, p);
+    }
+    GX_CHECK_LAUNCH("gx_slot_head_bwd_rows");
+    return GX_OK;
+}
+
+}
diff --git a/genesis_amd/functions.py b/genesis_amd/functions.py
--- a/genesis_amd/functions.py
+++ b/genesis_amd/functions.py
@@ -999,6 +999,37 @@
                 _ret(outs[2], dbe), None)
 
 
+def slot_head_fusable(S, wf, w1, w3):
+    return hip.slot_head_eligible(S, wf.view(wf.shape[0], -1), w1, w3)
+
+
+@ctx_bound
+class SlotHeadFn(torch.autograd.Function):
+
+    @staticmethod
+    def forward(ctx, S, msum, wf, fbias, gamma, beta, eps, w1, b1, w3, b3, noise):
+        S3, msum1, noise = S.contiguous(), msum.contiguous().view(-1), noise.contiguous()
+        res = hip.slot_head_fwd(S3, msum1, wf.view(wf.shape[0], -1), fbias, gamma, beta, eps, w1, b1, w3, b3, noise)
+        lin, stats, y, h1, zh, z, mu, sigma, log_q = res
+        ctx.save_for_backward(S3, msum1, noise, lin, stats, y, h1, zh)
+        ctx.params = (wf, fbias, gamma, beta, w1, b1, w3, b3)
+        ctx.msum_shape = msum.shape
+        ctx.set_materialize_grads(False)
+        return z, z.view(z.shape), mu, sigma, log_q
+
+    @staticmethod
+    def backward(ctx, gz, gz2, gmu, gsigma, glogq):
+        S3, msum1, noise, lin, stats, y, h1, zh = ctx.saved_tensors
+        wf, fbias, gamma, beta, w1, b1, w3, b3 = ctx.params
+        outs = tuple(_gout(p) for p in ctx.params)
+        res = hip.slot_head_bwd(S3, msum1, wf.view(wf.shape[0], -1), fbias, gamma, w1, w3, noise, lin, stats, y, h1, zh,
+                                _c(gz), _c(gz2), _c(gmu), _c(gsigma), _c(glogq), out=outs)
+        dS, dmsum = res[0], res[1].view(ctx.msum_shape)
+        dwf = res[2].view(wf.shape)
+        grads = [_ret(o, v) for o, v in zip(outs, (dwf,) + tuple(res[3:]))]
+        return (dS, dmsum, grads[0], grads[1], grads[2], grads[3], None, grads[4], grads[5], grads[6], grads[7], None)
+
+
 @ctx_bound
 class SBPScanFn(torch.autograd.Function):
 
diff --git a/genesis_amd/genesisv2_config.py b/genesis_amd/genesisv2_config.py
--- a/genesis_amd/genesisv2_config.py
+++ b/genesis_amd/genesisv2_config.py
@@ -273,16 +273,20 @@
         if f is None:
             f = fn.ConvGNReLUFn.apply(enc_feat, *self.feat_head[0].params())
         S, msum = fn.MaskPoolFn.apply(f, log_m)
-        ln = self.z_head[0]
-        zh = fn.PooledHeadFn.apply(fn.linear(S, self.feat_head[1].weight), msum, self.feat_head[1].bias,
-                                   ln.weight, ln.bias, ln.eps)
+        ln, fh, zh1, zh3 = self.z_head[0], self.feat_head[1], self.z_head[1], self.z_head[3]
         if eps is None:
             eps = torch.randn(K, B, D, device=dev)
-        zh = fn.linear(zh, self.z_head[1].weight, self.z_head[1].bias, 'relu')
-        zh = fn.linear(zh, self.z_head[3].weight, self.z_head[3].bias)
-        z, mu, sigma, log_q = fn.PosteriorFn.apply(zh, eps)
+        if fn.slot_head_fusable(S, fh.weight, zh1.weight, zh3.weight):
+            z, z_prior, mu, sigma, log_q = fn.SlotHeadFn.apply(S, msum, fh.weight, fh.bias, ln.weight, ln.bias, ln.eps,
+                                                               zh1.weight, zh1.bias, zh3.weight, zh3.bias, eps)
+        else:
+            zh = fn.PooledHeadFn.apply(fn.linear(S, fh.weight), msum, fh.bias, ln.weight, ln.bias, ln.eps)
+            zh = fn.linear(zh, zh1.weight, zh1.bias, 'relu')
+            zh = fn.linear(zh, zh3.weight, zh3.bias)
+            z, mu, sigma, log_q = fn.PosteriorFn.apply(zh, eps)
+            z_prior = z
         err, recon, x_r, log_m_r = self._decode(z, x, self.klm_loss and not self.detach_mr_in_klm)
-        kl = self._component_kl(z, log_q)
+        kl = self._component_kl(z_prior, log_q)
         t = dict(err=err, kl=kl, recon=recon, log_m=log_m, log_s=log_s, x_r=x_r, log_m_r=log_m_r, colour=colour, seeds=seeds,
                  idx=idx, mu=mu, sigma=sigma, z=z)
         if self.klm_loss:
diff --git a/genesis_amd/hip_ops.py b/genesis_amd/hip_ops.py
--- a/genesis_amd/hip_ops.py
+++ b/genesis_amd/hip_ops.py
@@ -1248,6 +1248,110 @@
     return dx, dw, db
 
 
+FUSE_SLOT_HEAD = os.environ.get('GENESIS_FUSE_SLOT_HEAD', '1') == '1'
+
+DJ_DW, DJ_COLS = 2, 3
+
+
+class DenseJob(ctypes.Structure):
+    _fields_ = [(n, ctypes.c_void_p) for n in ('a', 'mask', 'b', 'c', 'rs', 'rs2')] + \
+               [(n, ctypes.c_int) for n in ('lda', 'ldb', 'ldc', 'I', 'J', 'Kc', 'kind', 'act')]
+
+
+def _ptr(t):
+    return None if t is None else t.data_ptr()
+
+
+def dense_job_dw(g, x, dw, db=None, db2=None, mask=None, accumulate=False):
+    M, N = g.shape
+    K = x.shape[1]
+    ldg = _rows(g, 'dense_job_dw.g')
+    if mask is not None and _rows(mask, 'dense_job_dw.mask') != ldg:
+        raise GenesisHipError('dense_job_dw: mask and g must share a row stride')
+    _chk(dw, 'dense_job_dw.dw'); _chk(db, 'dense_job_dw.db'); _chk(db2, 'dense_job_dw.db2')
+    return DenseJob(_ptr(g), _ptr(mask), _ptr(x), _ptr(dw), _ptr(db), _ptr(db2 if db is not None else None), ldg,
+                    _rows(x, 'dense_job_dw.x'), K, N, K, M, DJ_DW, 10 if accumulate else 0), (g, x, dw, db, db2, mask)
+
+
+def dense_job_cols(cols, R, C, dgamma, dbeta, dfbias):
+    for t, n in ((dgamma, 'dgamma'), (dbeta, 'dbeta'), (dfbias, 'dfbias')):
+        _chk(t, 'dense_job_cols.' + n)
+    return DenseJob(_ptr(cols), None, None, _ptr(dgamma), _ptr(dbeta), _ptr(dfbias), 3 * C, 0, 0, R, C, 0, DJ_COLS, 0), \
+        (cols, dgamma, dbeta, dfbias)
+
+
+def dense_multi(jobs):
+    arr = (DenseJob * len(jobs))(*[j for j, _ in jobs])
+    _lib.call('gx_dense_multi', ctypes.cast(arr, ctypes.c_void_p), len(jobs), _stream())
+
+
+def _al16(*ts):
+    return all(t is None or t.data_ptr() % 16 == 0 for t in ts)
+
+
+def slot_head_eligible(S, wf, w1, w3):
+    if not FUSE_SLOT_HEAD or S.dim() != 3 or w3.shape[0] % 2:
+        return False
+    B, K, Cin = S.shape
+    C, N1, D = wf.shape[0], w1.shape[0], w3.shape[0] // 2
+    if wf.shape[1] != Cin or w1.shape[1] != C or w3.shape[1] != N1:
+        return False
+    return bool(_lib.query('gx_slot_head_eligible', B, K, Cin, C, N1, D)) and _al16(S, wf, w1, w3)
+
+
+def slot_head_fwd(S, msum, wf, fbias, gamma, beta, eps, w1, b1, w3, b3, noise):
+    for t, n in ((S, 'S'), (msum, 'msum'), (wf, 'wf'), (fbias, 'fbias'), (gamma, 'gamma'), (beta, 'beta'), (w1, 'w1'),
+                 (b1, 'b1'), (w3, 'w3'), (b3, 'b3'), (noise, 'noise')):
+        _chk(t, 'slot_head.' + n)
+    B, K, Cin = S.shape
+    C, N1, D = wf.shape[0], w1.shape[0], w3.shape[0] // 2
+    if tuple(noise.shape) != (K, B, D) or msum.numel() != B * K:
+        raise GenesisHipError('slot_head_fwd: noise must be [K,B,D] = %s and msum [B,K], got %s / %s'
+                              % ((K, B, D), tuple(noise.shape), tuple(msum.shape)))
+    dev, R = S.device, B * K
+    lin = torch.empty(R, C, dtype=F32, device=dev)
+    y = torch.empty(R, C, dtype=F32, device=dev)
+    stats = torch.empty(R, 2, dtype=F32, device=dev)
+    h1 = torch.empty(R, N1, dtype=F32, device=dev)
+    zh = torch.empty(B, K, 2 * D, dtype=F32, device=dev)
+    z = torch.empty(K, B, D, dtype=F32, device=dev)
+    mu, sigma = torch.empty_like(z), torch.empty_like(z)
+    log_q = torch.empty(K, B, dtype=F32, device=dev)
+    _lib.call('gx_slot_head_fwd', _p(S), _p(msum), _p(wf), _p(fbias), _p(gamma), _p(beta), float(eps), _p(w1), _p(b1), _p(w3),
+              _p(b3), _p(noise), B, K, Cin, C, N1, D, _p(lin), _p(stats), _p(y), _p(h1), _p(zh), _p(z), _p(mu), _p(sigma),
+              _p(log_q), _stream())
+    _probe_act(h1, b1, 'relu')
+    return lin, stats, y, h1, zh, z, mu, sigma, log_q
+
+
+def slot_head_bwd(S, msum, wf, fbias, gamma, w1, w3, noise, lin, stats, y, h1, zh, gz, gz2, gmu, gsigma, glogq,
+                  out=(None,) * 8):
+    for t, n in ((gz, 'gz'), (gz2, 'gz2'), (gmu, 'gmu'), (gsigma, 'gsigma'), (glogq, 'glogq')):
+        _chk(t, 'slot_head_bwd.' + n)
+    B, K, Cin = S.shape
+    C, N1, D = wf.shape[0], w1.shape[0], w3.shape[0] // 2
+    dev, R = S.device, B * K
+    dzh = torch.empty(R, 2 * D, dtype=F32, device=dev)
+    dh1 = torch.empty(R, N1, dtype=F32, device=dev)
+    dy = torch.empty(R, C, dtype=F32, device=dev)
+    dlin = torch.empty(R, C, dtype=F32, device=dev)
+    dmsum = torch.empty(R, dtype=F32, device=dev)
+    dS = torch.empty(B, K, Cin, dtype=F32, device=dev)
+    nb = _lib.query('gx_slot_head_bwd_ws_bytes', B, K, C)
+    ws = _ws(nb, dev)
+    _lib.call('gx_slot_head_bwd_rows', _p(zh), _p(noise), _p(gz), _p(gz2), _p(gmu), _p(gsigma), _p(glogq), _p(w3), _p(h1),
+              _p(w1), _p(lin), _p(msum), _p(fbias), _p(gamma), _p(stats), _p(wf), B, K, Cin, C, N1, D, _p(dzh), _p(dh1),
+              _p(dy), _p(dlin), _p(dmsum), _p(dS), _p(ws), nb, _stream())
+    shapes = ((C, Cin), (C,), (C,), (C,), (N1, C), (N1,), (2 * D, N1), (2 * D,))
+    dwf, dfb, dga, dbe, dw1, db1, dw3, db3 = [o if o is not None else torch.empty(s, dtype=F32, device=dev)
+                                              for o, s in zip(out, shapes)]
+    dense_multi([dense_job_dw(dzh, h1, dw3, db3),
+                 dense_job_dw(dh1, y, dw1, db1, mask=h1),
+                 dense_job_dw(dlin, S.view(R, Cin), dwf.view(C, Cin)),
+                 dense_job_cols(ws, R, C, dga, dbe, dfb)])
+    return dS, dmsum, dwf, dfb, dga, dbe, dw1, db1, dw3, db3
+
+
 def matmul_nn_fwd(x, w):
     _chk(x, 'matmul_nn.x'); _chk(w, 'matmul_nn.w')
     M, K = x.shape
diff --git a/include/genesis_hip.h b/include/genesis_hip.h
--- a/include/genesis_hip.h
+++ b/include/genesis_hip.h
@@ -322,6 +322,31 @@
                      float* dx, int lddx, int dx_accumulate, float* dw, float* db, float* db2, int M, int N, int K,
                      gx_stream_t stream);
 
+#define GX_DJ_DW 2
+#define GX_DJ_COLS 3
+typedef struct gx_dense_job {
+    const float* a;
+    const float* mask;
+    const float* b;
+    float* c;
+    float* rs;
+    float* rs2;
+    int lda, ldb, ldc, I, J, Kc, kind, act;
+} gx_dense_job;
+int gx_dense_multi(const gx_dense_job* jobs, int njobs, gx_stream_t stream);
+
+int gx_slot_head_eligible(int B, int K, int Cin, int C, int N1, int D);
+int gx_slot_head_fwd(const float* S, const float* msum, const float* wf, const float* fbias, const float* gamma,
+                     const float* beta, float eps, const float* w1, const float* b1, const float* w3, const float* b3,
+                     const float* noise, int B, int K, int Cin, int C, int N1, int D, float* lin, float* stats, float* y,
+                     float* h1, float* zh, float* z, float* mu, float* sigma, float* log_q, gx_stream_t stream);
+size_t gx_slot_head_bwd_ws_bytes(int B, int K, int C);
+int gx_slot_head_bwd_rows(const float* zh, const float* noise, const float* gz, const float* gz2, const float* gmu,
+                          const float* gsigma, const float* glogq, const float* w3, const float* h1, const float* w1,
+                          const float* lin, const float* msum, const float* fbias, const float* gamma, const float* stats,
+                          const float* wf, int B, int K, int Cin, int C, int N1, int D, float* dzh, float* dh1, float* dy,
+                          float* dlin, float* dmsum, float* dS, void* ws, size_t ws_bytes, gx_stream_t stream);
+
 int gx_matmul_nn_fwd(const float* x, const float* w, float* y, int M, int N, int K, gx_stream_t stream);
 size_t gx_matmul_nn_bwd_ws_bytes(int M, int N, int K);
 int gx_matmul_nn_bwd(const float* x, const float* w, const float* g, float* dx, float* dw, int M, int N, int K,
```

After: 12340 (median of 6 runs). No clear change (+0.4%).
